# anitasyang/Laplace-GNN

Measured on AMD Instinct MI355X. Metric: la.fit() samples/sec (GCN, KFAC), higher is better.
Workload: dtype f32; 1 GPU; arxiv-shaped 2-layer GCN, hessian_structure=kron (BASELINE configs[2]); num_nodes=169343, nnz=2501719, features=128, hidden=256, classes=40, n_train=90941, batch_size=10000, batches=10, parallelism=dp1 ((batch, class) units, contiguous balanced runs)

## Files before the change

laplace-gnn_amd/csrc/batchcache.hip:

```cpp
#include "lgnn_internal.h"

#include <algorithm>
#include <cstdlib>

namespace lgnn {

namespace {

constexpr size_t kSeenMax = 256;

void free_entry_memory(BatchEntry* e) {
  const uint64_t tag = e->tag;
  const int64_t M = e->M;
  *e = BatchEntry{};
  e->tag = tag;
  e->M = M;
}

void remove_entry(lgnn_ctx* h, BatchEntry* e) {
  BatchCache& c = h->bcache;
  c.bytes -= e->bytes;
  c.entries.erase(std::find(c.entries.begin(), c.entries.end(), e));
  delete e;
}

bool make_room(lgnn_ctx* h, BatchEntry* e, size_t add, size_t budget) {
  BatchCache& c = h->bcache;
  if (e->bytes + add > budget) return false;
  while (c.bytes + add > budget) {
    BatchEntry* lru = nullptr;
    for (BatchEntry* o : c.entries)
      if (o != e && o->bytes > 0 && (!lru || o->last_use < lru->last_use)) lru = o;
    if (!lru) return false;
    remove_entry(h, lru);
  }
  return true;
}

template <class T>
int alloc_copy(DevArray<T>& dst, const void* src, size_t count, hipStream_t s) {
  dst = {};
  const size_t bytes = std::max<size_t>(count, 1) * sizeof(T);
  if (hipMalloc(&dst.buf.p, bytes) != hipSuccess) {
    (void)hipGetLastError();
    dst.buf.p = nullptr;
    return 1;
  }
  dst.buf.bytes = bytes;
  if (count > 0) LGNN_HIP_CHECK(hipMemcpyAsync(dst.buf.p, src, count * sizeof(T), hipMemcpyDeviceToDevice, s));
  return 0;
}

void refuse(lgnn_ctx* h, BatchEntry* e) {
  h->bcache.bytes -= e->bytes;
  free_entry_memory(e);
  e->refused = true;
}

}

size_t batch_cache_budget() {
  const char* e = getenv("LGNN_BATCH_CACHE_MB");
  const long long mb = e ? atoll(e) : 2048;
  return mb <= 0 ? 0 : size_t(mb) << 20;
}

void batch_cache_clear(lgnn_ctx* h) {
  BatchCache& c = h->bcache;
  for (BatchEntry* e : c.entries) delete e;
  c.entries.clear();
  c.seen.clear();
  c.bytes = 0;
}

void batch_cache_drop_tag(lgnn_ctx* h, uint64_t tag) {
  BatchCache& c = h->bcache;
  for (BatchEntry* e : c.entries)
    if (e->tag == tag) { remove_entry(h, e); break; }
  c.seen.erase(std::remove(c.seen.begin(), c.seen.end(), tag), c.seen.end());
}

int batch_cache_lookup(lgnn_ctx* h, uint64_t tag, const int64_t* idx, int64_t M, BatchEntry** out, hipStream_t s) {
  *out = nullptr;
  BatchCache& c = h->bcache;
  if (tag == 0) return 0;
  const size_t budget = batch_cache_budget();
  if (budget == 0) {
    if (!c.entries.empty() || !c.seen.empty()) batch_cache_clear(h);
    return 0;
  }
  while (c.bytes > budget) {
    BatchEntry* lru = nullptr;
    for (BatchEntry* o : c.entries)
      if (o->bytes > 0 && (!lru || o->last_use < lru->last_use)) lru = o;
    if (!lru) break;
    remove_entry(h, lru);
  }
  for (BatchEntry* e : c.entries)
    if (e->tag == tag) {
      if (e->M != M) { remove_entry(h, e); break; }
      if (e->refused) return 0;
      e->last_use = ++c.clock;
      *out = e;
      return 0;
    }
  auto it = std::find(c.seen.begin(), c.seen.end(), tag);
  if (it == c.seen.end()) {
    if (c.seen.size() >= kSeenMax) c.seen.erase(c.seen.begin());
    c.seen.push_back(tag);
    return 0;
  }
  c.seen.erase(it);
  BatchEntry* e = new (std::nothrow) BatchEntry();
  if (!e) return 0;
  e->tag = tag;
  e->M = M;
  e->last_use = ++c.clock;
  c.entries.push_back(e);
  const size_t add = size_t(M) * 8;
  if (!make_room(h, e, add, budget) || alloc_copy(e->ids, idx, size_t(M), s) != 0) { refuse(h, e); return 0; }
  e->bytes += add;
  c.bytes += add;
  *out = e;
  return 0;
}

int batch_cache_store_active(lgnn_ctx* h, BatchEntry* e, hipStream_t s) {
  if (e->has_act || e->refused) return 0;
  const int64_t N = h->N;
  int32_t n = 0;
  LGNN_HIP_CHECK(hipMemcpyAsync(&n, h->ws.act_count.p, 4, hipMemcpyDeviceToHost, s));
  LGNN_HIP_CHECK(hipStreamSynchronize(s));
  LGNN_REQUIRE(n >= 0 && n <= N, "internal: active-row count out of range");
  const size_t add = size_t(N) + size_t(std::max(n, 1)) * 4 + 4;
  if (!make_room(h, e, add, batch_cache_budget()) || alloc_copy(e->active, h->ws.active.p, size_t(N), s) != 0 ||
      alloc_copy(e->act_list, h->ws.act_list.p, size_t(n), s) != 0 ||
      alloc_copy(e->act_count, h->ws.act_count.p, 1, s) != 0) {
    refuse(h, e);
    return 0;
  }
  e->bytes += add;
  h->bcache.bytes += add;
  e->has_act = true;
  return 0;
}

int batch_cache_store_paths(lgnn_ctx* h, BatchEntry* e, int64_t cap, bool have_nodes, hipStream_t s) {
  if (e->has_paths || e->refused) return 0;
  const int64_t N = h->N;
  Workspace& ws = h->ws;
  int32_t cnt[3] = {0, 0, 0};
  LGNN_HIP_CHECK(hipMemcpyAsync(&cnt[0], ws.path_pptr.as<int32_t>() + N, 4, hipMemcpyDeviceToHost, s));
  LGNN_HIP_CHECK(hipMemcpyAsync(&cnt[1], ws.path_rptr.as<int32_t>() + N, 4, hipMemcpyDeviceToHost, s));
  if (have_nodes) LGNN_HIP_CHECK(hipMemcpyAsync(&cnt[2], ws.path_nnodes.p, 4, hipMemcpyDeviceToHost, s));
  LGNN_HIP_CHECK(hipStreamSynchronize(s));
  const size_t np = (cnt[0] >= 0 && int64_t(cnt[0]) <= cap) ? size_t(cnt[0]) : 0;
  LGNN_REQUIRE(cnt[1] >= 0 && int64_t(cnt[1]) <= std::max<int64_t>(h->nnz, 1) && cnt[2] >= 0 && cnt[2] <= N,
               "internal: path structure counts out of range");
  const size_t nr = size_t(cnt[1]), nn = size_t(cnt[2]);
  size_t add = size_t(N + 1) * 4 + std::max<size_t>(np, 1) * 12;
  add += size_t(N + 1) * 4 + std::max<size_t>(nr, 1) * 8;
  if (have_nodes) add += std::max<size_t>(nn, 1) * 4 + 4;
  bool ok = make_room(h, e, add, batch_cache_budget());
  ok = ok && alloc_copy(e->pptr, ws.path_pptr.p, size_t(N + 1), s) == 0 && alloc_copy(e->pm, ws.path_pm.p, np, s) == 0 &&
       alloc_copy(e->pv, ws.path_pv.p, np, s) == 0 && alloc_copy(e->pw, ws.path_pw.p, np, s) == 0;
  if (ok)
    ok = alloc_copy(e->rptr, ws.path_rptr.p, size_t(N + 1), s) == 0 && alloc_copy(e->r_m, ws.path_rm.p, nr, s) == 0 &&
         alloc_copy(e->r_w, ws.path_rw.p, nr, s) == 0;
  if (ok && have_nodes)
    ok = alloc_copy(e->nodes, ws.path_nodes.p, nn, s) == 0 && alloc_copy(e->nnodes, ws.path_nnodes.p, 1, s) == 0;
  if (!ok) { refuse(h, e); return 0; }
  e->bytes += add;
  h->bcache.bytes += add;
  e->path_bytes = add;
  e->cap = cap;
  e->has_nodes = have_nodes;
  e->has_paths = true;
  return 0;
}

int batch_cache_store_pairs(lgnn_ctx* h, BatchEntry* e, hipStream_t s) {
  if (e->has_pairs || e->pairs_refused || e->refused || !e->has_paths) return 0;
  const int64_t N = h->N;
  Workspace& ws = h->ws;
  int32_t np = 0;
  LGNN_HIP_CHECK(hipMemcpyAsync(&np, ws.pair_ptr.as<int32_t>() + N, 4, hipMemcpyDeviceToHost, s));
  LGNN_HIP_CHECK(hipStreamSynchronize(s));
  LGNN_REQUIRE(np >= 0 && size_t(np) * 4 <= ws.pair_m.bytes, "internal: pair count out of range");
  const size_t M = size_t(e->M), add = M * 4 + std::max<size_t>(size_t(np), 1) * 12 + 4;
  const bool ok = make_room(h, e, add, batch_cache_budget()) && alloc_copy(e->pair_s, ws.pair_s.p, M, s) == 0 &&
                  alloc_copy(e->pair_m, ws.pair_m.p, size_t(np), s) == 0 && alloc_copy(e->pair_m2, ws.pair_m2.p, size_t(np), s) == 0 &&
                  alloc_copy(e->pair_w, ws.pair_w.p, size_t(np), s) == 0 &&
                  alloc_copy(e->pair_n, ws.pair_ptr.as<int32_t>() + N, 1, s) == 0;
  if (!ok) {
    e->pair_s = {}; e->pair_m = {}; e->pair_m2 = {}; e->pair_w = {}; e->pair_n = {};
    e->pairs_refused = true;
    return 0;
  }
  e->bytes += add;
  h->bcache.bytes += add;
  e->path_bytes += add;
  e->has_pairs = true;
  return 0;
}

void batch_cache_drop_paths(lgnn_ctx* h, BatchEntry* e) {
  if (!e->has_paths) return;
  e->pair_s = {}; e->pair_m = {}; e->pair_m2 = {}; e->pair_w = {}; e->pair_n = {};
  e->has_pairs = e->pairs_refused = false;
  e->pptr = {}; e->pm = {}; e->pv = {}; e->pw = {}; e->nodes = {}; e->nnodes = {}; e->rptr = {}; e->r_m = {}; e->r_w = {};
  e->has_paths = e->has_nodes = false;
  h->bcache.bytes -= e->path_bytes;
  e->bytes -= e->path_bytes;
  e->path_bytes = 0;
}

}

using namespace lgnn;

extern "C" int lgnn_kfac_batch_tag(lgnn_ctx* h, uint64_t tag) {
  if (!h) { set_error("null context"); return 2; }
  h->bcache.pending_tag = tag;
  return 0;
}

extern "C" int lgnn_batch_cache_drop(lgnn_ctx* h, uint64_t tag) {
  if (!h) { set_error("null context"); return 2; }
  if (tag == 0) batch_cache_clear(h);
  else batch_cache_drop_tag(h, tag);
  return 0;
}

extern "C" int lgnn_batch_cache_stats(const lgnn_ctx* h, int64_t* out) {
  if (!h || !out) { set_error("null argument"); return 2; }
  const BatchCache& c = h->bcache;
  int64_t n = 0;
  for (const BatchEntry* e : c.entries) n += e->bytes > 0 ? 1 : 0;
  out[0] = n; out[1] = int64_t(c.bytes); out[2] = c.hits; out[3] = c.misses; out[4] = c.builds;
  return 0;
}
```

laplace-gnn_amd/csrc/lgnn_internal.h:

```cpp
#pragma once
#include <atomic>
#include <cstring>
#include <hip/hip_runtime.h>
#include <stdint.h>
#include <string>
#include <type_traits>
#include <vector>

#include "../../include/laplace_gnn_hip.h"

namespace lgnn {

void set_error(const std::string& msg);

#define LGNN_HIP_CHECK(expr)                                                              \
  do {                                                                                    \
    hipError_t _e = (expr);                                                               \
    if (_e != hipSuccess) {                                                               \
      lgnn::set_error(std::string(#expr) + ": " + hipGetErrorString(_e));                 \
      return 1;                                                                           \
    }                                                                                     \
  } while (0)

#define LGNN_REQUIRE(cond, msg)                                                           \
  do {                                                                                    \
    if (!(cond)) {                                                                        \
      lgnn::set_error(std::string(msg) + " (" #cond ")");                                 \
      return 2;                                                                           \
    }                                                                                     \
  } while (0)

#define LGNN_CALL(expr)                                                                   \
  do {                                                                                    \
    int _rc = (expr);                                                                     \
    if (_rc != 0) return _rc;                                                             \
  } while (0)

inline int64_t cdiv(int64_t a, int64_t b) { return (a + b - 1) / b; }

template <auto Kernel>
int lds_opt_in(int bytes) {
  static std::atomic<uint64_t> done{0};
  int dev = 0;
  LGNN_HIP_CHECK(hipGetDevice(&dev));
  const uint64_t bit = dev < 64 ? uint64_t(1) << dev : 0;
  if (done.load(std::memory_order_acquire) & bit) return 0;
  LGNN_HIP_CHECK(hipFuncSetAttribute(reinterpret_cast<const void*>(Kernel), hipFuncAttributeMaxDynamicSharedMemorySize, bytes));
  done.fetch_or(bit, std::memory_order_release);
  return 0;
}

struct DevBuf {
  void* p = nullptr;
  size_t bytes = 0;
  bool host = false;
  DevBuf() = default;
  ~DevBuf();
  DevBuf(const DevBuf&) = delete;
  DevBuf& operator=(const DevBuf&) = delete;
  DevBuf(DevBuf&& o) noexcept;
  DevBuf& operator=(DevBuf&& o) noexcept;
  int reserve(size_t want);
  int reserve_host(size_t want);
  void release();
  template <class T> T* as() const { return reinterpret_cast<T*>(p); }
};
static_assert(!std::is_copy_constructible_v<DevBuf>);

struct Csr {
  int32_t* rowptr = nullptr;
  int32_t* col = nullptr;
  float* val = nullptr;
};

constexpr int kMaxLayers = 8;

struct ForwardCache {
  bool valid = false;
  bool aux_valid = false;
  bool wt_valid = false;
  bool x_valid = false;
  bool px_valid = false;
  DevBuf Xpad;
  int64_t prop_ld[kMaxLayers] = {};
  bool gram_valid[kMaxLayers] = {};
  DevBuf lin_in[kMaxLayers];
  DevBuf act_out[kMaxLayers];
  const float* lin_in_p[kMaxLayers] = {};
  int64_t lin_in_ld[kMaxLayers] = {};
  const float* hact_p[kMaxLayers] = {};
  int64_t hact_ld[kMaxLayers] = {};
  DevBuf out;
  DevBuf tmp;
  DevBuf gram_raw[kMaxLayers];
  DevBuf prop_in[kMaxLayers];
  DevBuf rowsum;
  DevBuf dact0;
  DevBuf mask_bits[kMaxLayers];
  DevBuf xhat[kMaxLayers];
  DevBuf rstd[kMaxLayers];
  DevBuf res_out;
  DevBuf pre_norm;
  template <class F> void each_buf(F&& f) const {
    for (int l = 0; l < kMaxLayers; ++l) {
      f(lin_in[l]); f(act_out[l]); f(gram_raw[l]); f(prop_in[l]); f(mask_bits[l]); f(xhat[l]); f(rstd[l]);
    }
    f(Xpad); f(out); f(tmp); f(rowsum); f(dact0); f(res_out); f(pre_norm);
  }
};

struct Workspace {
  DevBuf pos;
  DevBuf seeds;
  DevBuf probs;
  DevBuf mult;
  DevBuf planes_a;
  const void* planes_a_zero_ptr = nullptr;
  size_t planes_a_zero_bytes = 0;
  DevBuf planes_b;
  DevBuf gram_scratch[kMaxLayers];
  DevBuf misc;
  DevBuf jac;
  DevBuf top;
  DevBuf active;
  DevBuf val_act;
  DevBuf act_list;
  DevBuf act_count;
  DevBuf select_tmp;
  DevBuf flags;
  DevBuf out_flags, out_list, out_count;
  DevBuf val_act2;
  DevBuf path_coef, path_up, path_bg, path_cnt, path_rptr, path_rm, path_rw, path_zeros;
  DevBuf path_alpha;
  DevBuf path_pcnt, path_pptr, path_pm, path_pv, path_pw;
  DevBuf path_flags, path_nodes, path_nnodes;
  DevBuf pair_s, pair_cnt, pair_ptr, pair_m, pair_m2, pair_w;
  DevBuf pair_part;
  bool path_zeros_set = false;
  DevBuf gram_scratch_res[kMaxLayers];
  DevBuf planes_c;
  DevBuf adj_z0;
  DevBuf adj_dir;
  DevBuf lora_rows, lora_cols, lora_state, lora_count, lora_part;
  DevBuf dense_stored;
  DevBuf dense_rows;
  DevBuf subnet_keys, subnet_ord, subnet_iota, subnet_tmp, subnet_plan, subnet_x;
  DevBuf gp_tab_a, gp_tab_b, gp_phi_a, gp_phi_b, gp_g, gp_kt, gp_s, gp_wpair, gp_part, gp_jac_a, gp_jac_b;
  DevBuf cov_phit_a, cov_phit_b, cov_phis, cov_t2, cov_va, cov_vb, cov_add, cov_small, cov_scr;
  DevBuf ggn_jac, ggn_u, ggn_wt, ggn_tmp;
  DevBuf ggn_q, ggn_qbar, ggn_part;
  DevBuf cand_rows, cand_ord, cand_iota, cand_tmp, cand_ptr;
  template <class F> void each_buf(F&& f) const {
    for (int l = 0; l < kMaxLayers; ++l) { f(gram_scratch[l]); f(gram_scratch_res[l]); }
    f(pos); f(seeds); f(probs); f(mult); f(planes_a); f(planes_b); f(misc); f(jac); f(top); f(active); f(val_act);
    f(act_list); f(act_count); f(select_tmp); f(flags); f(out_flags); f(out_list); f(out_count); f(val_act2);
    f(path_coef); f(path_up); f(path_bg); f(path_cnt); f(path_rptr); f(path_rm); f(path_rw); f(path_zeros); f(path_alpha);
    f(path_pcnt); f(path_pptr); f(path_pm); f(path_pv); f(path_pw); f(path_flags); f(path_nodes); f(path_nnodes);
    f(pair_s); f(pair_cnt); f(pair_ptr); f(pair_m); f(pair_m2); f(pair_w); f(pair_part);
    f(planes_c); f(adj_z0); f(adj_dir); f(lora_rows); f(lora_cols); f(lora_state); f(lora_count); f(lora_part);
    f(dense_stored); f(dense_rows);
    f(subnet_keys); f(subnet_ord); f(subnet_iota); f(subnet_tmp); f(subnet_plan); f(subnet_x);
    f(gp_tab_a); f(gp_tab_b); f(gp_phi_a); f(gp_phi_b); f(gp_g); f(gp_kt); f(gp_s); f(gp_wpair); f(gp_part); f(gp_jac_a);
    f(gp_jac_b); f(cov_phit_a); f(cov_phit_b); f(cov_phis); f(cov_t2); f(cov_va); f(cov_vb); f(cov_add); f(cov_small);
    f(cov_scr); f(ggn_jac); f(ggn_u); f(ggn_wt); f(ggn_tmp); f(ggn_q); f(ggn_qbar); f(ggn_part);
    f(cand_rows); f(cand_ord); f(cand_iota); f(cand_tmp); f(cand_ptr);
  }
};

template <class T>
struct DevArray {
  DevBuf buf;
  operator T*() const { return buf.as<T>(); }
};
struct BatchEntry {
  uint64_t tag = 0;
  int64_t M = 0;
  uint64_t last_use = 0;
  size_t bytes = 0, path_bytes = 0;
  bool refused = false;
  DevArray<int64_t> ids;
  bool has_act = false;
  DevArray<uint8_t> active;
  DevArray<int32_t> act_list;
  DevArray<int32_t> act_count;
  bool has_paths = false;
  int64_t cap = 0;
  DevArray<int32_t> pptr;
  DevArray<int32_t> pm;
  DevArray<int32_t> pv;
  DevArray<float> pw;
  bool has_nodes = false;
  DevArray<int32_t> nodes;
  DevArray<int32_t> nnodes;
  DevArray<int32_t> rptr;
  DevArray<int32_t> r_m;
  DevArray<float> r_w;
  bool has_pairs = false;
  bool pairs_refused = false;
  DevArray<float> pair_s;
  DevArray<int32_t> pair_m;
  DevArray<int32_t> pair_m2;
  DevArray<float> pair_w;
  DevArray<int32_t> pair_n;
};
struct BatchCache {
  std::vector<BatchEntry*> entries;
  std::vector<uint64_t> seen;
  uint64_t pending_tag = 0;
  uint64_t clock = 0;
  size_t bytes = 0;
  int64_t hits = 0, misses = 0, builds = 0;
};

struct TrainState {
  bool tape_valid = false;
  bool input_valid = false;
  int64_t M = 0;
  float scale = 1.f;
  const uint8_t* masks[kMaxLayers] = {};
  DevBuf in[kMaxLayers];
  DevBuf xhat[kMaxLayers];
  DevBuf rstd[kMaxLayers];
  DevBuf out;
  DevBuf z, res;
  DevBuf ga, gb;
  DevBuf keys, keys_sorted, ord, ord_sorted, sort_tmp;
  DevBuf part;
  DevBuf wstack;
  DevBuf norm_part;
  template <class F> void each_buf(F&& f) const {
    for (int l = 0; l < kMaxLayers; ++l) { f(in[l]); f(xhat[l]); f(rstd[l]); }
    f(out); f(z); f(res); f(ga); f(gb); f(keys); f(keys_sorted); f(ord); f(ord_sorted); f(sort_tmp);
    f(part); f(wstack); f(norm_part);
  }
};

struct SampledState {
  bool in_valid = false;
  int64_t ldk = 0;
  DevBuf in0;
  DevBuf need;
  DevBuf rows;
  DevBuf count;
  DevBuf rpos;
  DevBuf z;
  DevBuf select_tmp;
  template <class F> void each_buf(F&& f) const {
    f(in0); f(need); f(rows); f(count); f(rpos); f(z); f(select_tmp);
  }
};

}

struct lgnn_ctx {
  int64_t N = 0;
  int64_t nnz = 0;
  int kind = 0;
  bool sym = false;
  bool self_loops = false;
  lgnn::Csr A, AT;
  lgnn::DevBuf A_rowptr, A_col, AT_rowptr, AT_col, val_fwd, val_bwd, deg_scale;
  lgnn::Csr P, PT;
  int L = 0;
  int64_t dims[lgnn::kMaxLayers + 1] = {};
  int64_t in_dim[lgnn::kMaxLayers] = {};
  const float* W[lgnn::kMaxLayers] = {};
  const float* b[lgnn::kMaxLayers] = {};
  const float* X = nullptr;
  int act = 0, lik = 0;
  int64_t n_params = 0;
  lgnn::DevBuf Wt[lgnn::kMaxLayers];
  bool has_res = false;
  int norm = 0;
  float norm_eps = 1e-5f;
  const float* Wr[lgnn::kMaxLayers] = {};
  const float* br[lgnn::kMaxLayers] = {};
  const float* norm_w[lgnn::kMaxLayers] = {};
  const float* norm_b[lgnn::kMaxLayers] = {};
  const float* norm_mean[lgnn::kMaxLayers] = {};
  const float* norm_var[lgnn::kMaxLayers] = {};
  lgnn::DevBuf Wrt[lgnn::kMaxLayers];
  lgnn::DevBuf Wcomb[lgnn::kMaxLayers], bcomb[lgnn::kMaxLayers];
  bool extras() const { return has_res || norm != 0; }
  int n_blocks() const { return has_res ? 2 * L - 1 : L; }
  const float* Wback(int l) const {
    return (has_res && kind == LGNN_KIND_SAGE && l < L - 1) ? Wcomb[l].as<float>() : W[l];
  }
  lgnn::ForwardCache fc;
  lgnn::Workspace ws;
  int64_t ws_limit = int64_t(32) << 30;
  int64_t cov_chunk_pairs = 0;
  bool last_route_paths = false;
  int last_top_kernel = 0;
  double two_hop_max = -1.0;
  double pair_hop_max = -1.0;
  double two_hop = -1.0;
  int64_t n_long = -1;
  int64_t n_long_tasks = 0;
  lgnn::DevBuf long_rows, long_slot, long_tasks, hub;
  lgnn::DevBuf top_multi, top_tasks, top_task_count, top_cnt, top_offs, top_hub_tiles;
  int64_t n_top_multi = 0, n_top_slices = 0;
  int64_t n_long_fwd = -1;
  lgnn::DevBuf long_rows_fwd;
  bool timing = false;
  std::vector<hipEvent_t> ev;
  size_t ev_used = 0;
  int64_t ev_planes = 0;
  lgnn::BatchCache bcache;
  lgnn::TrainState tr;
  lgnn::SampledState sf;
  template <class F> void each_buf(F&& f) const {
    for (int l = 0; l < lgnn::kMaxLayers; ++l) { f(Wt[l]); f(Wrt[l]); f(Wcomb[l]); f(bcomb[l]); }
    f(A_rowptr); f(A_col); f(AT_rowptr); f(AT_col); f(val_fwd); f(val_bwd); f(deg_scale);
    f(long_rows); f(long_slot); f(long_tasks); f(hub); f(long_rows_fwd);
    f(top_multi); f(top_tasks); f(top_task_count); f(top_cnt); f(top_offs); f(top_hub_tiles);
    fc.each_buf(f); ws.each_buf(f); tr.each_buf(f); sf.each_buf(f);
  }
  ~lgnn_ctx();
};

namespace lgnn {

struct SpmmArgs {
  const int32_t* rowptr;
  const int32_t* col;
  const float* val;
  int64_t nrows;
  const float* in;
  int64_t in_ld;
  int64_t in_plane_stride;
  float* out;
  int64_t out_ld;
  int64_t out_plane_stride;
  int64_t width;
  const float* self;
  int64_t self_ld;
  int64_t self_plane_stride;
  const float* hact;
  int64_t hact_ld;
  int act;
  int out_act;
  const int32_t* long_rows; int64_t n_long;
  bool skip_zero;
};

struct FusedArgs {
  const int32_t* rowptr; const int32_t* col; const float* val;
  int64_t nrows;
  int64_t nplanes;
  const float* in; int64_t in_ld; int64_t in_plane_stride;
  float* store; int64_t store_ld; int64_t store_plane_stride;
  const float* self; int64_t self_ld; int64_t self_plane_stride;
  const float* hact; int64_t hact_ld; int act;
  const uint8_t* self_rows; const uint32_t* mask_bits; int mask_words;
  int64_t width;
  float* scratch;
  int unused_;
  const int32_t* long_slot; const float* hub; int64_t hub_plane_stride; int64_t n_long;
  const int32_t* row_list; const int32_t* row_count;
};

struct BackGemmArgs {
  const float* G;
  const float* W;
  int64_t ldw;
  float* U;
  int64_t u_plane_stride;
  int64_t N, K, Nout;
  int64_t planes;
  const int32_t* rows;
  const int32_t* na_dev;
  const uint32_t* mask_bits; int64_t mask_words;
  const float* hact; int64_t hact_ld; int act;
};
bool backgemm_supported(int64_t K, int64_t Nout, bool with_mask);
int launch_backgemm(const BackGemmArgs& g, hipStream_t s);
int launch_relu_mask_bits(const float* h, int64_t ld, int64_t N, int64_t H, uint32_t* bits, hipStream_t s);
int compact_flags(const uint8_t* flags, int64_t n, int32_t* out, int32_t* count_dev, DevBuf& tmp, hipStream_t s);
int compact_rows(lgnn_ctx* h, const uint8_t* flags, DevBuf& list, DevBuf& count, hipStream_t s);
int compact_active_rows(lgnn_ctx* h, hipStream_t s);
int kfac_top_planes(lgnn_ctx* h, const int64_t* idx, int64_t M, bool fork_exact, float* g, hipStream_t s);
int exclusive_scan_i32(int32_t* in, int32_t* out, int64_t n, DevBuf& tmp, hipStream_t s);

int graph_build(lgnn_ctx* h, const int64_t* edge_index, int64_t E, hipStream_t s);
int graph_values(lgnn_ctx* h, bool same, hipStream_t s);
int graph_update(lgnn_ctx* h, const int64_t* fi, const int64_t* fj, const uint8_t* st, int64_t K, hipStream_t s);

struct DenseNtArgs {
  float* out = nullptr;
  int64_t ldo = 0, ncols = 0, nrows = 0;
  const int32_t* nrows_dev = nullptr;
  const int32_t* orows = nullptr;
  const int32_t* lrows = nullptr;
  const float* L = nullptr;
  int64_t l_ld = 0, l_stride = 0;
  const float* R = nullptr;
  int64_t r_ld = 0, r_stride = 0;
  int64_t width = 0, nplanes = 1;
  const float* rowc = nullptr;
  int64_t rowc_ld = 0;
};
int launch_dense_nt(const DenseNtArgs& g, hipStream_t s);
int launch_dense_diag_pair(const int64_t* idx, int64_t m0, int64_t mc, int64_t N, const int32_t* pos, const int32_t* mult,
                           const float* mask, int64_t H, const float* PX, int64_t ldx, const float* rowsum, int64_t F,
                           const float* H1p, int64_t ldh, const float* T, const float* phibar, float* out, hipStream_t s);
int launch_gp_rowcol(lgnn_ctx* h, const float* gP, float* rs, float* cs, hipStream_t s);
int dense_adj_finish(lgnn_ctx* h, float* G, hipStream_t s);

int launch_spmm(const Csr& m, int64_t nrows, const float* in, int64_t in_ld, float* out, int64_t out_ld,
                int64_t width, int epilogue, hipStream_t s, const int32_t* long_rows = nullptr, int64_t n_long = 0);
int launch_csr_rowsum(const Csr& m, int64_t nrows, float* out, hipStream_t s);

struct GemmEpilogue {
  const float* bias = nullptr;
  const float* hact = nullptr;
  int64_t hact_ld = 0;
  int act = 0;
  int64_t hact_row_mod = 0;
  int out_act = -1;
  const uint8_t* row_active = nullptr;
  bool no_atomics = false;
};
int launch_gemm(const float* A, int64_t lda, const float* B, int64_t ldb, float* C, int64_t ldc, int64_t R,
                int64_t K, int64_t Nout, const GemmEpilogue& ep, hipStream_t s);
int launch_gemm_devrows(const float* A, int64_t lda, const float* B, int64_t ldb, float* C, int64_t ldc, int64_t rows_bound,
                        const int32_t* r_dev, int64_t r_mul, int64_t K, int64_t Nout, float alpha, hipStream_t s);
int launch_gemm_listed(const float* A, int64_t lda, const float* B, int64_t ldb, float* C, int64_t ldc, int64_t planes,
                       int64_t plane_rows, const int32_t* list, const int32_t* na_dev, int64_t K, int64_t Nout,
                       const GemmEpilogue& ep, hipStream_t s);

int launch_gram(const float* X, int64_t ld, int64_t R, int64_t D, float* scratch, hipStream_t s);
int launch_gram_scaled(const float* X, int64_t ld, int64_t R, int64_t D, float* out, float scale, hipStream_t s);
int launch_gram_batched(const float* X, int64_t ld, int64_t R, int64_t D, float* out, int64_t out_zstride, int64_t nz,
                        const float* row_scale, const float* zscale, float scale, hipStream_t s);
int launch_symmetrize_upper(float* H, int64_t D, hipStream_t s);
int launch_sym_accumulate(const float* scratch, int64_t D, float scale, float* out, hipStream_t s, int64_t scratch_ld = 0);
int launch_spmm_ex(const SpmmArgs& a, int64_t nplanes, hipStream_t s);
int launch_spmm_gram_ex(const FusedArgs& a, hipStream_t s);
int launch_spmm_gram256(const FusedArgs& a, hipStream_t s);
bool fused_supported(int64_t width, int64_t in_ld, int64_t in_plane_stride, const void* in, int64_t rows);
int launch_spmm_gram(const Csr& m, int64_t nrows, int64_t nplanes, const float* in, float* store_or_null,
                     int64_t width, float* scratch, hipStream_t s);

int launch_transpose(const float* in, int64_t rows, int64_t cols, float* out, hipStream_t s);
int launch_act_deriv(const float* h, int64_t ld, int64_t N, int64_t H, int act, float* out, hipStream_t s);
int launch_fill_i32(int32_t* p, int64_t n, int32_t v, hipStream_t s);
int launch_gather_rows(const float* in, int64_t ld, int64_t nrows_in, const int64_t* idx, int64_t M, int64_t width,
                       float* out, int* bad_flag, hipStream_t s);

int launch_norm_forward(lgnn_ctx* h, int layer, const float* spre, int64_t s_ld, float* out, int64_t out_ld, hipStream_t s);
int launch_resnorm_backward(lgnn_ctx* h, int layer, float* U, int64_t ld, int64_t rows, const float* add, bool mask,
                            hipStream_t s);
int build_sage_res_weights(lgnn_ctx* h, int layer, hipStream_t s);
constexpr int kLongRow = 64;
constexpr int kTopSlice = 128;
int long_rows_ensure(lgnn_ctx* h, hipStream_t s);
int long_rows_fwd_ensure(lgnn_ctx* h, hipStream_t s);
int launch_long_rows_spmm(lgnn_ctx* h, const float* val, const float* in, int64_t in_ld, int64_t in_plane_stride,
                          int64_t nplanes, int64_t width, hipStream_t s);
struct KfacPlan {
  bool seeds_on_the_fly;
  bool sage_compact;
  bool need_pong;
  bool paths;
  bool fuse[kMaxLayers];
  bool backgemm[kMaxLayers];
  int64_t maxw, cc_max;
};
KfacPlan plan_kfac(int kind, int L, int64_t N, int64_t nnz, const int64_t* dims, int act, bool no_fuse, int64_t ws_limit,
                   bool no_paths = false);
struct KfacFisherOpts {
  const void* y_seed;
  float resid_scale;
  float b_scale;
  bool add_loss_and_A;
};
struct KfacShare { int64_t begin, end, count; };
int kfac_accumulate(lgnn_ctx* h, const int64_t* idx, const void* y, int64_t M, int64_t n_train, uint32_t flags,
                    int64_t class_begin, int64_t class_end, float* const* A_out, float* const* B_out, float* loss_out,
                    hipStream_t s, const KfacFisherOpts* fisher = nullptr, const KfacShare* share = nullptr);
int batch_prologue(lgnn_ctx* h, const int64_t* idx, const void* y, int64_t M, bool want_seeds, bool fork_exact,
                   float* loss_out, hipStream_t s, const void* y_seed = nullptr, float resid_scale = 1.0f,
                   const int64_t* guard_ids = nullptr);
int batch_epilogue(lgnn_ctx* h, const int64_t* idx, int64_t M, hipStream_t s);
int record_event(lgnn_ctx* h, hipStream_t s);
size_t batch_cache_budget();
void batch_cache_clear(lgnn_ctx* h);
int batch_cache_lookup(lgnn_ctx* h, uint64_t tag, const int64_t* idx, int64_t M, BatchEntry** out, hipStream_t s);
int batch_cache_store_active(lgnn_ctx* h, BatchEntry* e, hipStream_t s);
int batch_cache_store_paths(lgnn_ctx* h, BatchEntry* e, int64_t cap, bool have_nodes, hipStream_t s);
int batch_cache_store_pairs(lgnn_ctx* h, BatchEntry* e, hipStream_t s);
void batch_cache_drop_paths(lgnn_ctx* h, BatchEntry* e);
int launch_gram256_stream(const float* Y, int64_t ld, int64_t rows, int64_t width, float* scratch, hipStream_t s,
                          const int32_t* gate = nullptr, int64_t gate_cap = 0);
bool paths_supported(int kind, int L, const int64_t* dims, int act, int64_t nnz);
int two_hop_ensure(lgnn_ctx* h, hipStream_t s);
bool paths_pay(const lgnn_ctx* h, int64_t M);
constexpr int kCoefStride = 64;
constexpr int kCoefRow = 256;
struct PathR { const int32_t* rptr; const int32_t* r_m; const float* r_w; };
int launch_top_tiles(lgnn_ctx* h, const PathR& r, int64_t M, int64_t cb, int64_t ce, const int32_t* act_list,
                     const int32_t* act_count, float* scratch, hipStream_t s);
struct TopPairs { const float* sq; const int32_t* pm; const int32_t* pm2; const float* pw; const int32_t* npairs; };
int64_t top_pairs_bound(const lgnn_ctx* h, int64_t M);
bool top_pairs_fit(const lgnn_ctx* h, int64_t M);
int build_top_pairs(lgnn_ctx* h, const int64_t* idx, int64_t M, const PathR& r, TopPairs& out, hipStream_t s);
int launch_top_pairs(lgnn_ctx* h, const TopPairs& p, int64_t M, int64_t cb, int64_t ce, float* scratch, hipStream_t s);
struct TopTilesReq { const int32_t* act_list; const int32_t* act_count; float* scratch; bool pairs; };
int kfac_paths_first_layer(lgnn_ctx* h, const int64_t* idx, int64_t M, int seed_mode, int64_t cb, int64_t ce, float* scratch,
                           hipStream_t s, int64_t nb = 0, int64_t ne = -1, BatchEntry* entry = nullptr, bool* built = nullptr,
                           const TopTilesReq* top = nullptr);
int kfac_paths_first_layer_sage(lgnn_ctx* h, const int64_t* idx, int64_t M, int seed_mode, int64_t cb, int64_t ce,
                                float* scratch, hipStream_t s, int64_t nb = 0, int64_t ne = -1);
int forward_ensure(lgnn_ctx* h, hipStream_t s);
int forward_ensure_grams(lgnn_ctx* h, hipStream_t s);
int forward_ensure_aux(lgnn_ctx* h, hipStream_t s);
int forward_input_view(lgnn_ctx* h, hipStream_t s);
int build_px(lgnn_ctx* h, hipStream_t s);
int ensure_wt(lgnn_ctx* h, hipStream_t s);
bool gcn2_small_forward_supported(const lgnn_ctx* h);
int gcn2_forward_through_px(lgnn_ctx* h, hipStream_t s);
int diag_accumulate(lgnn_ctx* h, const int64_t* idx, const void* y, int64_t M, uint32_t flags, float* diag_out,
                    float* loss_out, hipStream_t s);
int lastlayer_full_accumulate(lgnn_ctx* h, const int64_t* idx, const void* y, int64_t M, float* H_out,
                              float* loss_out, hipStream_t s);
int lastlayer_pairs_accumulate(lgnn_ctx* h, const int64_t* idx, const void* y, int64_t M, float* S, float* Sb,
                               float* loss_out, hipStream_t s);
int lastlayer_features(lgnn_ctx* h, const int64_t* idx, int64_t M, float* out, float* f_out, hipStream_t s);
int lastlayer_pairs_place(lgnn_ctx* h, const float* S, const float* Sb, float* H_out, hipStream_t s);
int ef_accumulate(lgnn_ctx* h, const int64_t* idx, const void* y_seed, const void* y_loss, int64_t M, float resid_scale,
                  float scale, float* diag_out, float* full_out, float* grads_out, float* loss_out, hipStream_t s);
int lastlayer_kron_accumulate(lgnn_ctx* h, const int64_t* idx, const void* y, int64_t M, int64_t n_train, uint32_t flags,
                              float* A_out, float* B_out, float* Bb_out, float* loss_out, hipStream_t s);
int lastlayer_diag_accumulate(lgnn_ctx* h, const int64_t* idx, const void* y, int64_t M, float* diag_out, float* loss_out,
                              hipStream_t s);
int jacobians(lgnn_ctx* h, const int64_t* idx, int64_t M, float* J, float* f_out, hipStream_t s);
int full_accumulate(lgnn_ctx* h, const int64_t* idx, const void* y, int64_t M, float* H_out, float* loss_out, hipStream_t s);
int jacobians_subset(lgnn_ctx* h, const int64_t* idx, int64_t M, const int64_t* subnet, int64_t S, float* J, float* f_out,
                     hipStream_t s);
int subnet_full_accumulate(lgnn_ctx* h, const int64_t* idx, const void* y, int64_t M, const int64_t* subnet, int64_t S,
                           float* H_out, float* loss_out, hipStream_t s);
int gp_kernel(lgnn_ctx* h, const int64_t* idx_a, int64_t Ma, const int64_t* idx_b, int64_t Mb, int flags, float* K, int64_t ldk,
              hipStream_t s);
int gp_jvp(lgnn_ctx* h, const int64_t* idx, int64_t M, const float* v, float* out, hipStream_t s);
int glm_covariance(lgnn_ctx* h, const int64_t* idx_a, int64_t Ma, const int64_t* idx_b, int64_t Mb, int n_blocks,
                   const float* const* QA, const float* const* QB, const float* const* S, int flags, float* K, int64_t ldk,
                   hipStream_t s);
struct NtProblem {
  const float* A; int64_t lda, a_bs;
  const float* B; int64_t ldb, b_bs;
  float* Out; int64_t ldo, o_es, o_bs;
  int64_t Ra, Rb, K, batch;
  int upper_only = 0;
};
int launch_nt_gemm(lgnn_ctx* h, const NtProblem& p, hipStream_t s);
int jvp_block(lgnn_ctx* h, const int64_t* idx, int64_t M, const float* V, int64_t k, float* out, hipStream_t s);
int ggn_matmat(lgnn_ctx* h, const int64_t* idx, const void* y, int64_t M, const float* V, int64_t k, int flags, float* G,
               float* loss_out, hipStream_t s);
int sampled_forward(lgnn_ctx* h, const int64_t* idx, int64_t M, const float* theta, int64_t S, uint32_t flags, float* out,
                    hipStream_t s);
int sampled_ensure_input(lgnn_ctx* h, hipStream_t s);
int sampled_needed_rows(lgnn_ctx* h, const int64_t* idx, int64_t M, hipStream_t s);
struct GatherArgs {
  const int64_t* idx; int64_t M, N;
  const int32_t* rowptr; const int32_t* col; const float* val;
  const int32_t* rpos;
  const float* z; int64_t rcap, Cz, C;
  int sage, cw;
  const float* theta; int64_t P, offb;
  int64_t ns;
  float* out;
};
int launch_sampled_gather(const GatherArgs& g, hipStream_t s);
constexpr int SBM = 64, SBH = 64, SBK = 64, SLDT = SBK + 1, SLDH = SBH + 1, SZW = 128;
struct FwdArgs {
  static constexpr bool linearised = true;
  const float* in0; int64_t ldk;
  const int32_t* rows; const int32_t* count;
  const float* theta; int64_t P;
  int64_t Fp, H;
  const float* dact; const float* h1; int64_t h1_ld;
  const float* W1; int64_t ld1, off1, C, Cz;
  float* z; int64_t rcap;
};
int launch_first_layer(const FwdArgs& a, bool two, int64_t ndir, hipStream_t s);
int launch_full_directions(const float* J, const float* Gamma, const int64_t* idx, const float* logits, int64_t N,
                           int64_t mc, int64_t C, int64_t P, float* R, float* Kn, hipStream_t s);
void* blas_handle(hipStream_t s);
int sgemm_rm(hipStream_t s, int64_t R, int64_t Nout, int64_t K, float alpha, const float* A, int64_t lda, const float* B,
             int64_t ldb, float beta, float* Cm, int64_t ldc);

}
```

laplace-gnn_amd/csrc/paths.h:

```cpp
#pragma once
#include "lgnn_internal.h"

namespace lgnn {

constexpr int kYRows = 48;
__device__ __forceinline__ int coef_slot(int rel) { return ((rel & 15) << 2) | (rel >> 4); }
__device__ __forceinline__ int slot_class(int slot) { return ((slot & 3) << 4) | (slot >> 2); }
using f32x4 = __attribute__((ext_vector_type(4))) float;

struct YArgs {
  const int32_t* rowptr; const int32_t* col; const float* val;
  const int32_t* rptr; const int32_t* r_m; const float* r_w;
  const int32_t* pptr; const int32_t* pm; const int32_t* pv; const float* pw;
  int64_t cap;
  const float* coef;
  const float* zeros;
  const float* bg;
  const uint32_t* mask;
  int mask_words;
  const float* W1;
  int w1_ld;
  float* Y;
  int64_t N, M;
  int64_t n0, n1;
  const int32_t* list;
  const int32_t* n_list;
  int H, c0, R;
  int cb;
  int64_t n_coef;
  int unused_;
  int no_bg;
  int gram_f32;
};
static_assert(sizeof(YArgs) == 240 && __builtin_offsetof(YArgs, no_bg) == 228, "YArgs: paths_fused_kernel's argument offsets");

struct PathLists {
  const int32_t* rptr; const int32_t* r_m; const float* r_w;
  const int32_t* pptr; const int32_t* pm; const int32_t* pv; const float* pw;
  const int32_t* nodes; const int32_t* nnodes;
};

int launch_paths_fused(lgnn_ctx* h, YArgs y, int64_t cb, int64_t ce, float* scratch, hipStream_t s);
int launch_paths_overflow(lgnn_ctx* h, YArgs y, int64_t cb, int64_t ce, float* scratch, hipStream_t s);

}
```

laplace-gnn_amd/csrc/paths.hip:

```cpp
#include "device_utils.h"
#include "paths.h"

namespace lgnn {

namespace {

__global__ __launch_bounds__(256) void path_tables_kernel(const float* __restrict__ probs, const float* __restrict__ logits,
                                                          const int64_t* __restrict__ idx, const int32_t* __restrict__ pos,
                                                          int64_t M, int64_t N, int C, int cb, int ce, int mode,
                                                          float* __restrict__ coef, float* __restrict__ up,
                                                          const float* __restrict__ W1, int H, float* __restrict__ bg) {
  const int lane = threadIdx.x & 63;
  const int64_t m = int64_t(blockIdx.x) * 4 + (threadIdx.x >> 6);
  if (m >= M) return;
  const int64_t n = idx[m];
  float* __restrict__ cm = coef + m * kCoefRow;
  float* __restrict__ um = up + m * C;
  float* __restrict__ pm = up + (M + m) * C;
  const bool own = n >= 0 && n < N && pos[n] == int32_t(m);
  float pk = 0.f, fk = 0.f;
  if (own && lane < C && mode != 2) { pk = probs[m * C + lane]; fk = logits[n * C + lane]; }
  const float mb = wave_sum(pk * fk);
  const float sp = sqrtf(pk), t = fk - mb;
  float al = 0.f, be = 0.f, ga = 0.f, u = 0.f;
  if (own && lane < C) {
    if (mode == 2) al = 1.41421356237309515f;
    else if (mode == 1) { al = sp * (1.f + 0.5f * t); be = sp; ga = 0.5f * sp * t; u = pk * (1.f + t); }
    else { al = sp; be = sp; u = pk; }
  }
  const int c = cb + slot_class(lane);
  const bool have = c < ce;
  const int src = have ? c : 0;
  const float sal = __shfl(al, src), sbe = __shfl(be, src), sga = __shfl(ga, src);
  cm[lane] = have ? sal : 0.f;
  cm[kCoefStride + lane] = have ? -sbe : 0.f;
  cm[2 * kCoefStride + lane] = have ? -sga : 0.f;
  cm[3 * kCoefStride + lane] = 0.f;
  if (lane < C) { um[lane] = u; pm[lane] = own ? pk : 0.f; }
  if (bg == nullptr) return;
  const bool colv = 4 * lane < H;
  f32x4 b4 = {0.f, 0.f, 0.f, 0.f}, g4 = {0.f, 0.f, 0.f, 0.f};
  if (own) {
    const float* __restrict__ w = W1 + (colv ? 4 * lane : 0);
    for (int c = 0; c < C; ++c) {
      const float uc = __int_as_float(__builtin_amdgcn_readlane(__float_as_int(u), c));
      const float pc = __int_as_float(__builtin_amdgcn_readlane(__float_as_int(pk), c));
      const f32x4 wc = *reinterpret_cast<const f32x4*>(w + int64_t(c) * H);
      b4 += uc * wc;
      g4 += pc * wc;
    }
  }
  if (colv) {
    *reinterpret_cast<f32x4*>(bg + m * H + 4 * lane) = b4;
    *reinterpret_cast<f32x4*>(bg + (M + m) * H + 4 * lane) = g4;
  }
}

template <bool FILL>
__global__ __launch_bounds__(256) void path_r_kernel(const int64_t* __restrict__ idx, int64_t M, int64_t N,
                                                     const int32_t* __restrict__ pos, const int32_t* __restrict__ mult,
                                                     const int32_t* __restrict__ rowptr, const int32_t* __restrict__ col,
                                                     const float* __restrict__ val, int32_t* __restrict__ cnt,
                                                     const int32_t* __restrict__ rptr, int32_t* __restrict__ r_m,
                                                     float* __restrict__ r_w) {
  const int lane = threadIdx.x & 63;
  const int64_t m = int64_t(blockIdx.x) * 4 + (threadIdx.x >> 6);
  if (m >= M) return;
  const int64_t u = idx[m];
  if (u < 0 || u >= N || pos[u] != int32_t(m)) return;
  const float tm = FILL ? float(mult[m]) : 0.f;
  const int32_t e = rowptr[u + 1];
  for (int32_t p = rowptr[u] + lane; p < e; p += 64) {
    const int32_t v = col[p];
    const int32_t k = atomicAdd(&cnt[v], 1);
    if constexpr (FILL) {
      const int32_t slot = rptr[v] + k;
      r_m[slot] = int32_t(m);
      r_w[slot] = val[p] * tm;
    }
  }
}

template <bool FILL>
__global__ __launch_bounds__(256) void path_list_kernel(const int32_t* __restrict__ rowptr, const int32_t* __restrict__ col,
                                                        const float* __restrict__ val, int64_t N,
                                                        const int32_t* __restrict__ rptr, const int32_t* __restrict__ r_m,
                                                        const float* __restrict__ r_w, int32_t* __restrict__ pcnt,
                                                        const int32_t* __restrict__ pptr, int64_t cap,
                                                        int32_t* __restrict__ pm, int32_t* __restrict__ pv,
                                                        float* __restrict__ pw) {
  const int lane = threadIdx.x & 63;
  const int64_t n = int64_t(blockIdx.x) * 4 + (threadIdx.x >> 6);
  if (n >= N) return;
  if constexpr (FILL) {
    if (int64_t(pptr[N]) > cap) return;
  }
  const int32_t s = rowptr[n], e = rowptr[n + 1];
  int32_t run = FILL ? pptr[n] : 0;
  for (int32_t base = s; base < e; base += 64) {
    int32_t v = 0, r0 = 0, cnt = 0;
    float pval = 0.f;
    if (base + lane < e) {
      v = col[base + lane];
      pval = val[base + lane];
      r0 = rptr[v];
      cnt = rptr[v + 1] - r0;
    }
    int incl = cnt;
#pragma unroll
    for (int o = 1; o < 64; o <<= 1) {
      const int t = __shfl_up(incl, o);
      if (lane >= o) incl += t;
    }
    if constexpr (FILL) {
      const int32_t off = run + incl - cnt;
      for (int k = 0; k < cnt; ++k) {
        pm[off + k] = r_m[r0 + k];
        pv[off + k] = v;
        pw[off + k] = pval * r_w[r0 + k];
      }
    }
    run += __shfl(incl, 63);
  }
  if (!FILL && lane == 0) pcnt[n] = run;
}

__global__ __launch_bounds__(256) void sage_path_tables_kernel(const float* __restrict__ probs, const float* __restrict__ logits,
                                                               const int64_t* __restrict__ idx, const int32_t* __restrict__ pos,
                                                               int64_t M, int64_t N, int C, int cb, int ce, int mode,
                                                               float* __restrict__ coef, float* __restrict__ up,
                                                               float* __restrict__ alpha) {
  const int lane = threadIdx.x & 63;
  const int64_t m = int64_t(blockIdx.x) * 4 + (threadIdx.x >> 6);
  if (m >= M + C) return;
  const int c = cb + slot_class(lane);
  const bool have = c < ce;
  if (m >= M) {
    float* __restrict__ cm = coef + (2 * M + (m - M)) * kCoefRow;
    cm[lane] = 0.f; cm[kCoefStride + lane] = (have && c == int(m - M)) ? 1.f : 0.f; cm[2 * kCoefStride + lane] = 0.f; cm[3 * kCoefStride + lane] = 0.f;
    return;
  }
  const int64_t n = idx[m];
  const bool own = n >= 0 && n < N && pos[n] == int32_t(m);
  float pk = 0.f, fk = 0.f;
  if (own && lane < C && mode != 2) { pk = probs[m * C + lane]; fk = logits[n * C + lane]; }
  const float mb = wave_sum(pk * fk);
  const float sp = sqrtf(pk), t = fk - mb;
  float al = 0.f, be = 0.f, ga = 0.f, u = 0.f;
  if (own && lane < C) {
    if (mode == 2) al = 1.41421356237309515f;
    else if (mode == 1) { al = sp * (1.f + 0.5f * t); be = sp; ga = 0.5f * sp * t; u = pk * (1.f + t); }
    else { al = sp; be = sp; u = pk; }
  }
  const int src = have ? c : 0;
  float sal = __shfl(al, src), sbe = __shfl(be, src), sga = __shfl(ga, src);
  if (!have) { sal = 0.f; sbe = 0.f; sga = 0.f; }
  float* __restrict__ cs = coef + (2 * m) * kCoefRow;
  float* __restrict__ cn = coef + (2 * m + 1) * kCoefRow;
  cs[lane] = 0.f; cs[kCoefStride + lane] = -sbe; cs[2 * kCoefStride + lane] = -sga; cs[3 * kCoefStride + lane] = 0.f;
  cn[lane] = sal; cn[kCoefStride + lane] = -sbe; cn[2 * kCoefStride + lane] = -sga; cn[3 * kCoefStride + lane] = 0.f;
  alpha[m * kCoefStride + lane] = al;
  if (lane < C) { up[m * C + lane] = u; up[(M + m) * C + lane] = own ? pk : 0.f; }
}

template <bool FILL>
__global__ __launch_bounds__(256) void sage_path_list_kernel(const int32_t* __restrict__ rowptr, const int32_t* __restrict__ col,
                                                             const float* __restrict__ val, int64_t N, int64_t M, int C,
                                                             const int32_t* __restrict__ pos, const int32_t* __restrict__ mult,
                                                             const float* __restrict__ alpha, int32_t* __restrict__ pcnt,
                                                             const int32_t* __restrict__ pptr, int32_t* __restrict__ pm,
                                                             int32_t* __restrict__ pv, float* __restrict__ pw) {
  const int lane = threadIdx.x & 63;
  const int64_t n = int64_t(blockIdx.x) * 4 + (threadIdx.x >> 6);
  if (n >= N) return;
  const int32_t s = rowptr[n], e = rowptr[n + 1];
  int32_t run = FILL ? pptr[n] : 0;
  for (int32_t base = s; base < e; base += 64) {
    int32_t mv = INT32_MAX;
    float w = 0.f;
    if (base + lane < e) { mv = pos[col[base + lane]]; w = val[base + lane]; }
    const bool in = mv != INT32_MAX;
    const uint64_t bal = __ballot(in);
    if constexpr (FILL) {
      if (in) {
        const int32_t o = run + __popcll(bal & ((uint64_t(1) << lane) - 1));
        pm[o] = 2 * mv + 1; pv[o] = int32_t(n); pw[o] = w * float(mult[mv]);
      }
    }
    run += __popcll(bal);
  }
  const int32_t ms = pos[n];
  if (ms != INT32_MAX) {
    if constexpr (FILL) {
      const float tm = float(mult[ms]);
      if (lane == 0) { pm[run] = 2 * ms; pv[run] = int32_t(n); pw[run] = tm; }
      if (lane < C) {
        pm[run + 1 + lane] = int32_t(2 * M) + lane; pv[run + 1 + lane] = int32_t(n);
        pw[run + 1 + lane] = tm * alpha[int64_t(ms) * kCoefStride + lane];
      }
    }
    run += 1 + C;
  }
  if (!FILL && lane == 0) pcnt[n] = run;
}

__global__ void path_flag_kernel(const int32_t* __restrict__ pptr, int64_t n0, int64_t n, uint8_t* __restrict__ flags) {
  const int64_t k = int64_t(blockIdx.x) * blockDim.x + threadIdx.x;
  if (k < n) flags[k] = pptr[n0 + k + 1] > pptr[n0 + k] ? 1 : 0;
}

__global__ void two_hop_count_kernel(const int32_t* __restrict__ rp, const int32_t* __restrict__ rpt, int64_t N,
                                     unsigned long long* __restrict__ out) {
  unsigned long long acc = 0;
  const int64_t stride = int64_t(gridDim.x) * blockDim.x;
  for (int64_t v = int64_t(blockIdx.x) * blockDim.x + threadIdx.x; v < N; v += stride)
    acc += (unsigned long long)(rp[v + 1] - rp[v]) * (unsigned long long)(rpt[v + 1] - rpt[v]);
  for (int o = 32; o > 0; o >>= 1) acc += __shfl_xor(acc, o);
  if ((threadIdx.x & 63) == 0 && acc) atomicAdd(out, acc);
}

__global__ void two_hop_max_kernel(const int32_t* __restrict__ rp, const int32_t* __restrict__ col,
                                   const int32_t* __restrict__ rp2, int64_t N, unsigned long long* __restrict__ out) {
  unsigned long long best = 0;
  const int64_t stride = int64_t(gridDim.x) * blockDim.x;
  for (int64_t m = int64_t(blockIdx.x) * blockDim.x + threadIdx.x; m < N; m += stride) {
    unsigned long long acc = 0;
    for (int32_t p = rp[m]; p < rp[m + 1]; ++p) { const int32_t k = col[p]; acc += (unsigned long long)(rp2[k + 1] - rp2[k]); }
    best = acc > best ? acc : best;
  }
  for (int o = 32; o > 0; o >>= 1) { const unsigned long long t = __shfl_xor(best, o); best = t > best ? t : best; }
  if ((threadIdx.x & 63) == 0 && best) atomicMax(out, best);
}
}

int two_hop_ensure(lgnn_ctx* h, hipStream_t s) {
  if (h->two_hop >= 0) return 0;
  h->two_hop = 0;
  if (h->nnz <= 0) return 0;
  DevBuf acc;
  LGNN_CALL(acc.reserve(64));
  unsigned long long host[3] = {0, 0, 0};
  LGNN_HIP_CHECK(hipMemsetAsync(acc.p, 0, 24, s));
  const dim3 grid{unsigned(std::min<int64_t>(cdiv(h->N, 256), 1024))};
  hipLaunchKernelGGL(two_hop_count_kernel, grid, dim3(256), 0, s, h->P.rowptr, h->PT.rowptr, h->N, acc.as<unsigned long long>());
  LGNN_HIP_CHECK(hipGetLastError());
  hipLaunchKernelGGL(two_hop_max_kernel, grid, dim3(256), 0, s, h->P.rowptr, h->P.col, h->P.rowptr, h->N,
                     acc.as<unsigned long long>() + 1);
  LGNN_HIP_CHECK(hipGetLastError());
  hipLaunchKernelGGL(two_hop_max_kernel, grid, dim3(256), 0, s, h->P.rowptr, h->P.col, h->PT.rowptr, h->N,
                     acc.as<unsigned long long>() + 2);
  LGNN_HIP_CHECK(hipGetLastError());
  LGNN_HIP_CHECK(hipMemcpyAsync(host, acc.p, 24, hipMemcpyDeviceToHost, s));
  LGNN_HIP_CHECK(hipStreamSynchronize(s));
  h->two_hop = double(host[0]);
  h->two_hop_max = double(host[1]);
  h->pair_hop_max = double(host[2]);
  return 0;
}
constexpr double kPathsPerNodeLimit = 24.0;
bool paths_pay(const lgnn_ctx* h, int64_t M) {
  const double N = double(h->N);
  return h->two_hop >= 0 && h->two_hop / N * double(M) / N <= kPathsPerNodeLimit;
}

bool paths_supported(int kind, int L, const int64_t* dims, int act, int64_t nnz) {
  const int64_t C = dims[L], H = L >= 2 ? dims[L - 1] : 0;
  return (kind == LGNN_KIND_GCN || kind == LGNN_KIND_SAGE) && L == 2 && act == LGNN_ACT_RELU && nnz > 0 && C <= kCoefStride &&
         H > 128 && H <= 256 && H % 4 == 0;
}

static int64_t path_list_cap(const lgnn_ctx* h) {
  int64_t cap = std::max<int64_t>(4 * h->nnz, int64_t(1) << 22);
  if (const char* e = getenv("LGNN_PATH_LIST_CAP")) cap = std::max<int64_t>(1, std::min<int64_t>(cap, atoll(e)));
  return cap;
}
bool top_pairs_fit(const lgnn_ctx* h, int64_t M) {
  int64_t cap = path_list_cap(h);
  if (const char* e = getenv("LGNN_PAIR_LIST_CAP")) cap = std::max<int64_t>(1, std::min<int64_t>(cap, atoll(e)));
  const int64_t bound = top_pairs_bound(h, M);
  return bound > 0 && bound <= cap;
}

static int path_node_list(lgnn_ctx* h, PathLists& pl, int64_t nb, int64_t ne, hipStream_t s) {
  Workspace& ws = h->ws;
  const int64_t n = ne - nb;
  LGNN_CALL(ws.path_flags.reserve(size_t(h->N)));
  LGNN_CALL(ws.path_nodes.reserve(size_t(h->N) * 4));
  LGNN_CALL(ws.path_nnodes.reserve(64));
  hipLaunchKernelGGL(path_flag_kernel, dim3(unsigned(cdiv(n, 256))), dim3(256), 0, s, pl.pptr, nb, n, ws.path_flags.as<uint8_t>());
  LGNN_HIP_CHECK(hipGetLastError());
  pl.nodes = ws.path_nodes.as<int32_t>(); pl.nnodes = ws.path_nnodes.as<int32_t>();
  return compact_flags(ws.path_flags.as<uint8_t>(), n, ws.path_nodes.as<int32_t>(), ws.path_nnodes.as<int32_t>(), ws.select_tmp, s);
}
static int path_list_reserve(lgnn_ctx* h, int64_t cap, PathLists& pl, hipStream_t s) {
  Workspace& ws = h->ws;
  LGNN_CALL(ws.path_pcnt.reserve(size_t(h->N + 1) * 4));
  LGNN_CALL(ws.path_pptr.reserve(size_t(h->N + 1) * 4));
  LGNN_CALL(ws.path_pm.reserve(size_t(cap) * 4));
  LGNN_CALL(ws.path_pv.reserve(size_t(cap) * 4));
  LGNN_CALL(ws.path_pw.reserve(size_t(cap) * 4));
  LGNN_HIP_CHECK(hipMemsetAsync(ws.path_pcnt.as<int32_t>() + h->N, 0, 4, s));
  pl.pptr = ws.path_pptr.as<int32_t>(); pl.pm = ws.path_pm.as<int32_t>(); pl.pv = ws.path_pv.as<int32_t>();
  pl.pw = ws.path_pw.as<float>();
  return 0;
}
static int path_zeros_ensure(Workspace& ws, hipStream_t s) {
  LGNN_CALL(ws.path_zeros.reserve(1024));
  if (!ws.path_zeros_set) LGNN_HIP_CHECK(hipMemsetAsync(ws.path_zeros.p, 0, 1024, s));
  ws.path_zeros_set = true;
  return 0;
}

static YArgs path_args(lgnn_ctx* h, const PathLists& pl, int64_t cb, int64_t cap, int64_t nb, int64_t ne) {
  YArgs y{};
  y.rowptr = h->PT.rowptr; y.col = h->PT.col; y.val = h->PT.val;
  y.rptr = pl.rptr; y.r_m = pl.r_m; y.r_w = pl.r_w;
  y.pptr = pl.pptr; y.pm = pl.pm; y.pv = pl.pv; y.pw = pl.pw; y.cap = cap;
  y.list = pl.nodes; y.n_list = pl.nnodes;
  y.coef = h->ws.path_coef.as<float>(); y.bg = h->ws.path_bg.as<float>(); y.zeros = h->ws.path_zeros.as<float>();
  y.mask = h->fc.mask_bits[0].as<uint32_t>(); y.mask_words = int(cdiv(h->dims[1], 32));
  y.N = h->N; y.n0 = nb; y.n1 = ne; y.H = int(h->dims[1]); y.cb = int(cb);
  return y;
}

int kfac_paths_first_layer(lgnn_ctx* h, const int64_t* idx, int64_t M, int seed_mode, int64_t cb, int64_t ce, float* scratch,
                           hipStream_t s, int64_t nb, int64_t ne, BatchEntry* entry, bool* built, const TopTilesReq* top) {
  const int64_t N = h->N, C = h->dims[2], H = h->dims[1];
  if (ne < 0) ne = N;
  LGNN_REQUIRE(nb >= 0 && nb <= ne && ne <= N, "internal: node range");
  if (nb == ne) return 0;
  Workspace& ws = h->ws;
  LGNN_REQUIRE(paths_supported(h->kind, h->L, h->dims, h->act, h->nnz), "internal: path route on an unsupported model");
  LGNN_CALL(ws.path_coef.reserve(size_t(M) * kCoefRow * 4));
  LGNN_CALL(ws.path_up.reserve(size_t(2 * M) * C * 4));
  LGNN_CALL(ws.path_bg.reserve(size_t(2 * M) * H * 4));
  const bool no_bg = seed_mode == 2;
  const bool bg_in_tables = !no_bg && (reinterpret_cast<uintptr_t>(h->W[1]) & 15) == 0;
  hipLaunchKernelGGL(path_tables_kernel, dim3(unsigned(cdiv(M, 4))), dim3(256), 0, s, ws.probs.as<float>(),
                     h->fc.out.as<float>(), idx, ws.pos.as<int32_t>(), M, N, int(C), int(cb), int(ce), seed_mode,
                     ws.path_coef.as<float>(), ws.path_up.as<float>(), h->W[1], int(H),
                     bg_in_tables ? ws.path_bg.as<float>() : static_cast<float*>(nullptr));
  LGNN_HIP_CHECK(hipGetLastError());
  if (!no_bg && !bg_in_tables) {
    GemmEpilogue none;
    LGNN_CALL(launch_gemm(ws.path_up.as<float>(), C, h->W[1], H, ws.path_bg.as<float>(), H, 2 * M, C, H, none, s));
  }
  const int64_t cap = path_list_cap(h);
  const bool can_overflow = !(h->two_hop_max >= 0 && double(M) * h->two_hop_max <= double(cap));
  const double ppn = h->two_hop >= 0 ? h->two_hop / double(N) * double(M) / double(N) : 1e9;
  const bool use_list = ppn < 2.5;
  const bool whole = nb == 0 && ne == N;
  LGNN_CALL(path_zeros_ensure(ws, s));
  if (entry && entry->refused) entry = nullptr;
  if (entry && entry->has_paths && entry->cap != cap) batch_cache_drop_paths(h, entry);
  const bool cached = entry && entry->has_paths;
  PathLists pl{};
  if (cached) {
    pl = {entry->rptr, entry->r_m, entry->r_w, entry->pptr, entry->pm, entry->pv, entry->pw, nullptr, nullptr};
  } else {
    LGNN_CALL(ws.path_cnt.reserve(size_t(N + 1) * 4));
    LGNN_CALL(ws.path_rptr.reserve(size_t(N + 1) * 4));
    LGNN_CALL(ws.path_rm.reserve(size_t(std::max<int64_t>(h->nnz, 1)) * 4));
    LGNN_CALL(ws.path_rw.reserve(size_t(std::max<int64_t>(h->nnz, 1)) * 4));
    LGNN_HIP_CHECK(hipMemsetAsync(ws.path_cnt.p, 0, size_t(N + 1) * 4, s));
    hipLaunchKernelGGL(path_r_kernel<false>, dim3(unsigned(cdiv(M, 4))), dim3(256), 0, s, idx, M, N, ws.pos.as<int32_t>(),
                       ws.mult.as<int32_t>(), h->P.rowptr, h->P.col, h->P.val, ws.path_cnt.as<int32_t>(),
                       static_cast<const int32_t*>(nullptr), static_cast<int32_t*>(nullptr), static_cast<float*>(nullptr));
    LGNN_HIP_CHECK(hipGetLastError());
    LGNN_CALL(exclusive_scan_i32(ws.path_cnt.as<int32_t>(), ws.path_rptr.as<int32_t>(), N + 1, ws.select_tmp, s));
    LGNN_HIP_CHECK(hipMemsetAsync(ws.path_cnt.p, 0, size_t(N + 1) * 4, s));
    hipLaunchKernelGGL(path_r_kernel<true>, dim3(unsigned(cdiv(M, 4))), dim3(256), 0, s, idx, M, N, ws.pos.as<int32_t>(),
                       ws.mult.as<int32_t>(), h->P.rowptr, h->P.col, h->P.val, ws.path_cnt.as<int32_t>(),
                       ws.path_rptr.as<int32_t>(), ws.path_rm.as<int32_t>(), ws.path_rw.as<float>());
    LGNN_HIP_CHECK(hipGetLastError());
    LGNN_CALL(path_list_reserve(h, cap, pl, s));
    const dim3 pgrid{unsigned(cdiv(N, 4))};
    hipLaunchKernelGGL(path_list_kernel<false>, pgrid, dim3(256), 0, s, h->PT.rowptr, h->PT.col, h->PT.val, N,
                       ws.path_rptr.as<int32_t>(), ws.path_rm.as<int32_t>(), ws.path_rw.as<float>(), ws.path_pcnt.as<int32_t>(),
                       static_cast<const int32_t*>(nullptr), cap, static_cast<int32_t*>(nullptr), static_cast<int32_t*>(nullptr),
                       static_cast<float*>(nullptr));
    LGNN_HIP_CHECK(hipGetLastError());
    LGNN_CALL(exclusive_scan_i32(ws.path_pcnt.as<int32_t>(), ws.path_pptr.as<int32_t>(), N + 1, ws.select_tmp, s));
    hipLaunchKernelGGL(path_list_kernel<true>, pgrid, dim3(256), 0, s, h->PT.rowptr, h->PT.col, h->PT.val, N,
                       ws.path_rptr.as<int32_t>(), ws.path_rm.as<int32_t>(), ws.path_rw.as<float>(), ws.path_pcnt.as<int32_t>(),
                       ws.path_pptr.as<int32_t>(), cap, ws.path_pm.as<int32_t>(), ws.path_pv.as<int32_t>(), ws.path_pw.as<float>());
    LGNN_HIP_CHECK(hipGetLastError());
    pl.rptr = ws.path_rptr.as<int32_t>(); pl.r_m = ws.path_rm.as<int32_t>(); pl.r_w = ws.path_rw.as<float>();
  }
  if (use_list) {
    if (cached && whole && entry->has_nodes) {
      pl.nodes = entry->nodes; pl.nnodes = entry->nnodes;
    } else {
      LGNN_CALL(path_node_list(h, pl, nb, ne, s));
    }
  }
  if (entry && !cached) {
    LGNN_CALL(batch_cache_store_paths(h, entry, cap, use_list && whole, s));
    if (built) *built = true;
  }
  if (top && top->pairs) {
    TopPairs tp{};
    if (entry && entry->has_pairs) {
      tp = {entry->pair_s, entry->pair_m, entry->pair_m2, entry->pair_w, entry->pair_n};
    } else {
      LGNN_CALL(build_top_pairs(h, idx, M, PathR{pl.rptr, pl.r_m, pl.r_w}, tp, s));
      if (entry && entry->has_paths) LGNN_CALL(batch_cache_store_pairs(h, entry, s));
    }
    LGNN_CALL(launch_top_pairs(h, tp, M, cb, ce, top->scratch, s));
  } else if (top) {
    LGNN_CALL(launch_top_tiles(h, PathR{pl.rptr, pl.r_m, pl.r_w}, M, cb, ce, top->act_list, top->act_count, top->scratch, s));
  }
  YArgs y = path_args(h, pl, cb, cap, nb, ne);
  y.W1 = h->W[1]; y.w1_ld = int(H); y.M = M; y.n_coef = M; y.no_bg = no_bg ? 1 : 0;
  LGNN_CALL(launch_paths_fused(h, y, cb, ce, scratch, s));
  return can_overflow ? launch_paths_overflow(h, y, cb, ce, scratch, s) : 0;
}

int kfac_paths_first_layer_sage(lgnn_ctx* h, const int64_t* idx, int64_t M, int seed_mode, int64_t cb, int64_t ce, float* scratch,
                                hipStream_t s, int64_t nb, int64_t ne) {
  const int64_t N = h->N, C = h->dims[2], H = h->dims[1];
  if (ne < 0) ne = N;
  LGNN_REQUIRE(nb >= 0 && nb <= ne && ne <= N, "internal: node range");
  if (nb == ne) return 0;
  Workspace& ws = h->ws;
  LGNN_REQUIRE(h->kind == LGNN_KIND_SAGE && paths_supported(h->kind, h->L, h->dims, h->act, h->nnz),
               "internal: path route on an unsupported model");
  const int64_t T = 2 * M + C;
  LGNN_CALL(ws.path_coef.reserve(size_t(T) * kCoefRow * 4));
  LGNN_CALL(ws.path_up.reserve(size_t(2 * M) * C * 4));
  LGNN_CALL(ws.path_bg.reserve(size_t(2 * T) * H * 4));
  LGNN_CALL(ws.path_alpha.reserve(size_t(M) * kCoefStride * 4));
  hipLaunchKernelGGL(sage_path_tables_kernel, dim3(unsigned(cdiv(M + C, 4))), dim3(256), 0, s, ws.probs.as<float>(),
                     h->fc.out.as<float>(), idx, ws.pos.as<int32_t>(), M, N, int(C), int(cb), int(ce), seed_mode,
                     ws.path_coef.as<float>(), ws.path_up.as<float>(), ws.path_alpha.as<float>());
  LGNN_HIP_CHECK(hipGetLastError());
  float* bg = ws.path_bg.as<float>();
  GemmEpilogue none;
  LGNN_CALL(launch_gemm(ws.path_up.as<float>(), C, h->W[1], 2 * H, bg, 2 * H, M, C, 2 * H, none, s));
  LGNN_CALL(launch_gemm(ws.path_up.as<float>() + M * C, C, h->W[1], 2 * H, bg + T * H, 2 * H, M, C, 2 * H, none, s));
  LGNN_HIP_CHECK(hipMemcpy2DAsync(bg + 2 * M * H, size_t(H) * 4, h->W[1], size_t(2 * H) * 4, size_t(H) * 4, size_t(C),
                                  hipMemcpyDeviceToDevice, s));
  LGNN_HIP_CHECK(hipMemsetAsync(bg + (T + 2 * M) * H, 0, size_t(C) * H * 4, s));
  LGNN_CALL(path_zeros_ensure(ws, s));
  const int64_t cap = std::max<int64_t>(h->nnz, 1) + (C + 1) * M + 64;
  LGNN_REQUIRE(cap < (int64_t(1) << 31), "too many paths for one launch");
  PathLists pl{};
  LGNN_CALL(path_list_reserve(h, cap, pl, s));
  const dim3 pgrid{unsigned(cdiv(N, 4))};
  hipLaunchKernelGGL(sage_path_list_kernel<false>, pgrid, dim3(256), 0, s, h->PT.rowptr, h->PT.col, h->PT.val, N, M, int(C),
                     ws.pos.as<int32_t>(), ws.mult.as<int32_t>(), ws.path_alpha.as<float>(), ws.path_pcnt.as<int32_t>(),
                     static_cast<const int32_t*>(nullptr), static_cast<int32_t*>(nullptr), static_cast<int32_t*>(nullptr),
                     static_cast<float*>(nullptr));
  LGNN_HIP_CHECK(hipGetLastError());
  LGNN_CALL(exclusive_scan_i32(ws.path_pcnt.as<int32_t>(), ws.path_pptr.as<int32_t>(), N + 1, ws.select_tmp, s));
  hipLaunchKernelGGL(sage_path_list_kernel<true>, pgrid, dim3(256), 0, s, h->PT.rowptr, h->PT.col, h->PT.val, N, M, int(C),
                     ws.pos.as<int32_t>(), ws.mult.as<int32_t>(), ws.path_alpha.as<float>(), ws.path_pcnt.as<int32_t>(),
                     ws.path_pptr.as<int32_t>(), ws.path_pm.as<int32_t>(), ws.path_pv.as<int32_t>(), ws.path_pw.as<float>());
  LGNN_HIP_CHECK(hipGetLastError());
  LGNN_CALL(path_node_list(h, pl, nb, ne, s));
  YArgs y = path_args(h, pl, cb, cap, nb, ne);
  y.W1 = h->W[1] + H; y.w1_ld = int(2 * H);
  y.M = T; y.n_coef = T; y.no_bg = 0;
  return launch_paths_fused(h, y, cb, ce, scratch, s);
}

}
```

laplace-gnn_amd/csrc/paths_fused.hip:

```cpp
#include "gram256.h"
#include "paths.h"

namespace lgnn {
namespace {

constexpr int kYStride = 272;
constexpr int kPlaneDwords = 512;
constexpr int kGroupDwords = 3 * kPlaneDwords;
constexpr int kYGroups = kYRows / 4;
__device__ __forceinline__ int piece_swap(int q) { return (q ^ (q >> 2)) & 1; }
__device__ __forceinline__ int piece_col(int c) { return 8 * (c >> 2) + 4 * (((c >> 1) & 1) ^ piece_swap(c >> 2)) + 2 * (c & 1); }

struct alignas(16) FusedShared {
  union {
    uint32_t pc[2][kYGroups][3][kPlaneDwords];
    float y[2][kYRows][kYStride];
  };
  int ready[4], done[4];
};
static_assert(sizeof(FusedShared) <= 160 * 1024, "the CU's LDS");

__device__ __forceinline__ int lds_min4(const int* c) {
  int4 v;
  asm volatile("ds_read_b128 %0, %1\n\ts_waitcnt lgkmcnt(0)" : "=v"(v) : "v"(uint32_t(reinterpret_cast<uintptr_t>(c))) : "memory");
  return __builtin_amdgcn_readfirstlane(min(min(v.x, v.y), min(v.z, v.w)));
}
__device__ __forceinline__ void lds_publish(int* c, int value, int lane) {
  if (lane == 0)
    asm volatile("ds_write_b32 %0, %1\n\ts_waitcnt lgkmcnt(0)" :: "v"(uint32_t(reinterpret_cast<uintptr_t>(c))), "v"(value) : "memory");
}

using i32x4 = int __attribute__((ext_vector_type(4)));
__device__ __forceinline__ i32x4 make_rsrc(const void* p, uint64_t bytes) {
  const uint64_t u = reinterpret_cast<uint64_t>(p);
  return i32x4{int(uint32_t(u)), int(uint32_t(u >> 32) & 0xffffu), int(uint32_t(bytes > 0xffffffffull ? 0xffffffffull : bytes)),
               0x00020000};
}
template <bool LIST>
struct NodeRanges {
  i32x4 prs, lrs;
  uint32_t r;
  int64_t base, cnt;
  uint32_t n0;
  __device__ __forceinline__ void init(const int32_t* __restrict__ pptr, const int32_t* __restrict__ list, int64_t n0_, int64_t N,
                                       int64_t nn, int64_t cnt_) {
    prs = make_rsrc(pptr, uint64_t(N + 1) * 4);
    lrs = make_rsrc(LIST ? list : pptr, uint64_t(LIST ? nn : 0) * 4);
    n0 = uint32_t(n0_); cnt = cnt_;
    fill(0);
  }
  __device__ __forceinline__ void fill(int64_t b) {
    base = b;
    const uint32_t ii = uint32_t(b) + (threadIdx.x & 31u);
    const bool in = int64_t(ii) < cnt;
    const uint32_t k = blockIdx.x + ii * gridDim.x;
    uint32_t node = k;
    if constexpr (LIST)
      asm volatile("buffer_load_dword %0, %1, %2, 0 offen\n\ts_waitcnt vmcnt(0)" : "=&v"(node) : "v"(in ? k * 4u : 0xfffffff0u), "s"(lrs) : "memory");
    const uint32_t off = in ? (n0 + node) * 4u + ((threadIdx.x >> 3) & 4u) : 0xfffffff0u;
    asm volatile("buffer_load_dword %0, %1, %2, 0 offen\n\ts_waitcnt vmcnt(0)" : "=&v"(r) : "v"(off), "s"(prs) : "memory");
  }
  __device__ __forceinline__ void get(int64_t i, int32_t& p0, int32_t& p1) {
    if (i - base >= 32) fill(i);
    const int l = int(i - base);
    p0 = __builtin_amdgcn_readlane(int(r), l); p1 = __builtin_amdgcn_readlane(int(r), l + 32);
  }
};

template <int OFF>
__device__ __forceinline__ void bload4(f32x4& d, uint32_t voff, const i32x4& rsrc) {
  asm volatile("buffer_load_dwordx4 %0, %1, %2, 0 offen offset:%3" : "=v"(d) : "v"(voff), "s"(rsrc), "n"(OFF) : "memory");
}
__device__ __forceinline__ void bload1(uint32_t& d, uint32_t voff, const i32x4& rsrc) {
  asm volatile("buffer_load_dword %0, %1, %2, 0 offen" : "=v"(d) : "v"(voff), "s"(rsrc) : "memory");
}
using bf16x8 = __attribute__((ext_vector_type(8))) __bf16;
using u32x4v = __attribute__((ext_vector_type(4))) uint32_t;
using u32x2v = __attribute__((ext_vector_type(2))) uint32_t;

__device__ __forceinline__ uint32_t pk_bf16(float lo, float hi) {
  using bf16x2 = __attribute__((ext_vector_type(2))) __bf16;
  const bf16x2 v = {static_cast<__bf16>(lo), static_cast<__bf16>(hi)};
  return __builtin_bit_cast(uint32_t, v);
}
__device__ __forceinline__ void split_pair(float ya, float yb, uint32_t& q0, uint32_t& q1, uint32_t& q2) {
  q0 = pk_bf16(ya, yb);
  asm("" : "+v"(q0));
  const float r1a = ya - __uint_as_float(q0 << 16), r1b = yb - __uint_as_float(q0 & 0xffff0000u);
  q1 = pk_bf16(r1a, r1b);
  asm("" : "+v"(q1));
  q2 = pk_bf16(r1a - __uint_as_float(q1 << 16), r1b - __uint_as_float(q1 & 0xffff0000u));
}

struct PTables {
  i32x4 coef, b, g, mask, pm, pv, pw;
};

struct PMeta { uint32_t oc, ob, om, w; };
__device__ __forceinline__ void meta_issue(const PTables& tb, int32_t p0, int32_t p1, int lane, PMeta& t) {
  const uint32_t q = uint32_t(max(min(p0 + lane, p1 - 1), 0)) * 4u;
  bload1(t.oc, q, tb.pm);
  bload1(t.om, q, tb.pv);
  bload1(t.w, q, tb.pw);
}
template <int YOUNGER>
__device__ __forceinline__ void meta_finish(int32_t p0, int32_t p1, int lane, uint32_t row_bytes, uint32_t mask_bytes, PMeta& t) {
  asm volatile("s_waitcnt vmcnt(%3)" : "+v"(t.oc), "+v"(t.om), "+v"(t.w) : "n"(YOUNGER) : "memory");
  const bool in = p0 + lane < p1;
  const uint32_t m = in ? t.oc : 0u, v = in ? t.om : 0u;
  t.oc = m * uint32_t(kCoefRow * 4); t.ob = m * row_bytes; t.om = v * mask_bytes;
  t.w = in ? t.w : 0u;
}

struct PLane {
  int kq;
  uint32_t oc, ob, om;
  int mshift;
};

struct POps {
  f32x4 ca[3];
  f32x4 b4, g4;
  uint32_t mw;
  float w;
};

template <bool NOBG> constexpr int kStepLoads = NOBG ? 2 : 6;
template <bool NOBG>
__device__ __forceinline__ void p_load(const PTables& tb, const PMeta& mt, int s, const PLane& pl, POps& o) {
  const int src = 4 * s + pl.kq;
  const uint32_t oc = uint32_t(__shfl(int(mt.oc), src)) + pl.oc;
  const uint32_t om = uint32_t(__shfl(int(mt.om), src)) + pl.om;
  o.w = __uint_as_float(uint32_t(__shfl(int(mt.w), src)));
  bload4<0>(o.ca[0], oc, tb.coef);
  if constexpr (!NOBG) {
    const uint32_t ob = uint32_t(__shfl(int(mt.ob), src)) + pl.ob;
    bload4<kCoefStride * 4>(o.ca[1], oc, tb.coef);
    bload4<2 * kCoefStride * 4>(o.ca[2], oc, tb.coef);
    bload4<0>(o.b4, ob, tb.b);
    bload4<0>(o.g4, ob, tb.g);
  }
  bload1(o.mw, om, tb.mask);
}
template <bool NOBG, int YOUNGER>
__device__ __forceinline__ void p_wait(POps& o) {
  if constexpr (NOBG)
    asm volatile("s_waitcnt vmcnt(%2)" : "+v"(o.ca[0]), "+v"(o.mw) : "n"(YOUNGER) : "memory");
  else
    asm volatile("s_waitcnt vmcnt(%6)" : "+v"(o.ca[0]), "+v"(o.ca[1]), "+v"(o.ca[2]), "+v"(o.b4), "+v"(o.g4), "+v"(o.mw)
                 : "n"(YOUNGER) : "memory");
}

struct PCur { float a1[3], a2[3], bb[4], gg[4]; };
struct PAlpha { u32x4v a[3], m[4]; };
constexpr uint32_t kHiHalves = 0x07060302u;
template <bool NOBG, bool HI, bool SB>
__device__ __forceinline__ void p_xform(const POps& o, const PLane& pl, PCur& c, PAlpha& al, bool bg) {
#pragma unroll
  for (int t = 0; t < 3; ++t) {
    const int tt = HI ? 3 : t;
    if (HI && t > 0) {
      if constexpr (!SB) al.a[t][0] = 0u;
      al.a[t][1] = 0u; al.a[t][2] = 0u;
      continue;
    }
    float av = o.w * o.ca[0][tt];
    asm("" : "+v"(av));
    const uint32_t h0 = __float_as_uint(av) & 0xffff0000u;
    const float r1 = av - __uint_as_float(h0);
    const float r2 = r1 - __uint_as_float(__float_as_uint(r1) & 0xffff0000u);
    if constexpr (!SB) {
      al.a[t][0] = __builtin_amdgcn_perm(__float_as_uint(r1), __float_as_uint(av), kHiHalves);
      al.a[t][1] = __float_as_uint(r2) >> 16;
    } else {
      al.a[t][1] |= h0;
      al.a[t][2] = __builtin_amdgcn_perm(__float_as_uint(r2), __float_as_uint(r1), kHiHalves);
    }
  }
  const int bits = int(o.mw >> pl.mshift);
#pragma unroll
  for (int ct = 0; ct < 4; ++ct) {
    const int on = __builtin_amdgcn_sbfe(bits, ct, 1);
    if constexpr (!SB) {
      al.m[ct][0] = uint32_t(on) & 0x3f803f80u;
      al.m[ct][1] = uint32_t(on) & 0x00003f80u;
    } else {
      al.m[ct][1] |= uint32_t(on) & 0x3f800000u;
      al.m[ct][2] = uint32_t(on) & 0x3f803f80u;
    }
  }
  if constexpr (!NOBG) {
    if (bg) {
#pragma unroll
      for (int t = 0; t < 3; ++t) {
        const int tt = HI ? 3 : t;
        c.a1[t] = (HI && t > 0) ? 0.f : o.w * o.ca[1][tt];
        c.a2[t] = (HI && t > 0) ? 0.f : o.w * o.ca[2][tt];
      }
#pragma unroll
      for (int ct = 0; ct < 4; ++ct) {
        const int on = __builtin_amdgcn_sbfe(bits, ct, 1);
        c.bb[ct] = __uint_as_float(uint32_t(on) & __float_as_uint(o.b4[ct]));
        c.gg[ct] = __uint_as_float(uint32_t(on) & __float_as_uint(o.g4[ct]));
      }
    }
  }
}
template <bool NOBG>
__device__ __forceinline__ void p_keep(const PCur& c) {
  if constexpr (!NOBG) {
    asm volatile("" :: "v"(c.a1[0]), "v"(c.a1[1]), "v"(c.a1[2]), "v"(c.a2[0]), "v"(c.a2[1]), "v"(c.a2[2]));
    asm volatile("" :: "v"(c.bb[0]), "v"(c.bb[1]), "v"(c.bb[2]), "v"(c.bb[3]), "v"(c.gg[0]), "v"(c.gg[1]), "v"(c.gg[2]), "v"(c.gg[3]));
  }
}
__device__ __forceinline__ f32x4 mfma_bf16(u32x4v a, u32x4v b, f32x4 c) {
  return __builtin_amdgcn_mfma_f32_16x16x32_bf16(__builtin_bit_cast(bf16x8, a), __builtin_bit_cast(bf16x8, b), c, 0, 0, 0);
}
__device__ __forceinline__ void p_mfma(const PCur& c, f32x4 (&y2)[3][4]) {
#pragma unroll
  for (int t = 0; t < 3; ++t)
#pragma unroll
    for (int ct = 0; ct < 4; ++ct) y2[t][ct] = __builtin_amdgcn_mfma_f32_16x16x4f32(c.a1[t], c.bb[ct], y2[t][ct], 0, 0, 0);
#pragma unroll
  for (int t = 0; t < 3; ++t)
#pragma unroll
    for (int ct = 0; ct < 4; ++ct) y2[t][ct] = __builtin_amdgcn_mfma_f32_16x16x4f32(c.a2[t], c.gg[ct], y2[t][ct], 0, 0, 0);
}
__device__ __forceinline__ void p_mfma_first(const PCur& c, f32x4 (&y2)[3][4]) {
  const f32x4 zero = {0.f, 0.f, 0.f, 0.f};
#pragma unroll
  for (int t = 0; t < 3; ++t)
#pragma unroll
    for (int ct = 0; ct < 4; ++ct) y2[t][ct] = __builtin_amdgcn_mfma_f32_16x16x4f32(c.a1[t], c.bb[ct], zero, 0, 0, 0);
#pragma unroll
  for (int t = 0; t < 3; ++t)
#pragma unroll
    for (int ct = 0; ct < 4; ++ct) y2[t][ct] = __builtin_amdgcn_mfma_f32_16x16x4f32(c.a2[t], c.gg[ct], y2[t][ct], 0, 0, 0);
}
template <bool FIRST>
__device__ __forceinline__ void p_mfma_alpha(const PAlpha& al, f32x4 (&t1)[3][4]) {
  const f32x4 zero = {0.f, 0.f, 0.f, 0.f};
#pragma unroll
  for (int t = 0; t < 3; ++t)
#pragma unroll
    for (int ct = 0; ct < 4; ++ct) t1[t][ct] = mfma_bf16(al.a[t], al.m[ct], FIRST ? zero : t1[t][ct]);
}

template <bool LIST>
struct ChunkGen {
  int64_t gi;
  int32_t gp, gend;
  int32_t pa0, pa1;
  NodeRanges<LIST> nr;
  __device__ __forceinline__ void init(const int32_t* __restrict__ pptr, const int32_t* __restrict__ list, int64_t n0, int64_t N,
                                       int64_t nn, int64_t cnt) {
    nr.init(pptr, list, n0, N, nn, cnt);
    gi = 0;
    nr.get(0, gp, gend);
    nr.get(1, pa0, pa1);
  }
  __device__ __forceinline__ void next(int64_t cnt, int32_t& q0, int32_t& q1, bool& last) {
    q0 = gp; q1 = min(gp + 64, gend);
    last = q1 >= gend;
    if (last) {
      ++gi;
      gp = pa0; gend = pa1;
      nr.get(gi + 1, pa0, pa1);
    } else {
      gp = q1;
    }
  }
};

template <bool NOBG, bool HI>
__device__ __forceinline__ void pair_body(const PTables& tb, const PMeta& mx, int sx, const PLane& pl, POps& A, POps& B, PCur& cA,
                                          PCur& cB, PAlpha& al, f32x4 (&t1)[3][4], f32x4 (&y2)[3][4], bool first, bool half) {
  constexpr int NL = kStepLoads<NOBG>;
  p_wait<NOBG, NL>(A);
  p_xform<NOBG, HI, false>(A, pl, cA, al, true);
  p_keep<NOBG>(cB);
  p_load<NOBG>(tb, mx, sx, pl, A);
  if constexpr (!NOBG) {
    if (first) p_mfma_first(cA, y2);
    else p_mfma(cA, y2);
  }
  p_wait<NOBG, NL>(B);
  p_xform<NOBG, HI, true>(B, pl, cB, al, !half);
  p_keep<NOBG>(cA);
  p_load<NOBG>(tb, mx, sx + 1, pl, B);
  if (first) p_mfma_alpha<true>(al, t1);
  else p_mfma_alpha<false>(al, t1);
  if constexpr (!NOBG)
    if (!half) p_mfma(cB, y2);
}
template <bool LIST, bool NOBG, bool HI>
__device__ __forceinline__ void product_role(const YArgs& a, const int32_t* __restrict__ pptr, const int32_t* __restrict__ list,
                                             FusedShared& sh, int64_t nn, int64_t cnt, int cg) {
  const int lane = threadIdx.x & 63;
  const int H = a.H;
  const bool path_wave = 64 * cg < H;
  if (!path_wave) return;
  PLane pl;
  const int li = lane & 15;
  pl.kq = lane >> 4;
  const int col = 64 * cg + 4 * li;
  const bool col_ok = col < H;
  pl.oc = 16u * uint32_t(li);
  pl.ob = col_ok ? 4u * uint32_t(col) : 0u;
  pl.om = col_ok ? 4u * uint32_t(col >> 5) : 0x7ffffff0u;
  pl.mshift = col & 31;
  const uint32_t row_bytes = uint32_t(H) * 4u, mask_bytes = uint32_t(a.mask_words) * 4u;
  PTables tb;
  tb.coef = make_rsrc(a.coef, uint64_t(a.n_coef) * kCoefRow * 4);
  tb.b = make_rsrc(a.bg, uint64_t(a.M) * row_bytes);
  tb.g = make_rsrc(a.bg + a.M * int64_t(H), uint64_t(a.M) * row_bytes);
  tb.mask = make_rsrc(a.mask, uint64_t(a.N) * mask_bytes);
  tb.pm = make_rsrc(a.pm, uint64_t(a.cap) * 4);
  tb.pv = make_rsrc(a.pv, uint64_t(a.cap) * 4);
  tb.pw = make_rsrc(a.pw, uint64_t(a.cap) * 4);
  const uint32_t w1_row_bytes = uint32_t(a.w1_ld) * 4u;
  const i32x4 w1rs = make_rsrc(a.W1 + int64_t(a.c0) * a.w1_ld, uint64_t(a.R - 1) * w1_row_bytes + row_bytes);
  constexpr int NL = kStepLoads<NOBG>;
  ChunkGen<LIST> gen;
  gen.init(pptr, list, a.n0, a.N, nn, cnt);
  int32_t q0c, q1c, q0n, q1n;
  bool lastc, lastn;
  gen.next(cnt, q0c, q1c, lastc);
  gen.next(cnt, q0n, q1n, lastn);
  PMeta mc, mn;
  meta_issue(tb, q0c, q1c, lane, mc);
  meta_issue(tb, q0n, q1n, lane, mn);
  meta_finish<0>(q0c, q1c, lane, row_bytes, mask_bytes, mc);
  meta_finish<0>(q0n, q1n, lane, row_bytes, mask_bytes, mn);
  POps A, B;
  p_load<NOBG>(tb, mc, 0, pl, A);
  p_load<NOBG>(tb, mc, 1, pl, B);
  f32x4 t1[3][4], y2[3][4];
#pragma unroll
  for (int t = 0; t < 3; ++t)
#pragma unroll
    for (int ct = 0; ct < 4; ++ct) { t1[t][ct] = f32x4{0.f, 0.f, 0.f, 0.f}; y2[t][ct] = f32x4{0.f, 0.f, 0.f, 0.f}; }
  PCur cA = {}, cB = {};
  PAlpha al;
#pragma unroll
  for (int t = 0; t < 3; ++t) al.a[t] = u32x4v{0u, 0u, 0u, 0u};
#pragma unroll
  for (int ct = 0; ct < 4; ++ct) al.m[ct] = u32x4v{0u, 0u, 0u, 0u};
  bool node_has = false;
  bool firstc = true;
  for (int64_t i = 0; i < cnt;) {
    int32_t q0f, q1f;
    bool lastf;
    gen.next(cnt, q0f, q1f, lastf);
    PMeta mf2;
    meta_issue(tb, q0f, q1f, lane, mf2);
    const int kch = q1c - q0c, np = max((kch + 7) >> 3, 1);
    node_has = node_has || kch > 0;
#pragma clang loop unroll(disable)
    for (int j = 0; j < np; ++j) {
      const bool more = j + 1 < np;
      PMeta mx;
      mx.oc = more ? mc.oc : mn.oc; mx.ob = more ? mc.ob : mn.ob; mx.om = more ? mc.om : mn.om; mx.w = more ? mc.w : mn.w;
      const int sx = more ? 2 * (j + 1) : 0;
      const bool first = firstc && j == 0, half = !more && 4 * (2 * j + 1) >= kch;
      pair_body<NOBG, HI>(tb, mx, sx, pl, A, B, cA, cB, al, t1, y2, first, half);
    }
    if (lastc) {
      int wl = lane;
      asm volatile("" : "+v"(wl));
      const int wkq = wl >> 4, wcol = 64 * cg + 4 * (wl & 15);
      const bool wcol_ok = wcol < H;
      const uint32_t w1_off = wcol_ok ? uint32_t(4 * wkq) * w1_row_bytes + 4u * uint32_t(wcol) : 0x7ff00000u;
      const int pc_lo = 8 * (wcol >> 2) + 4 * piece_swap(wcol >> 2), pc_hi = pc_lo ^ 4;
      f32x4 w1[3][4];
#pragma unroll
      for (int t = 0; t < 3; ++t)
#pragma unroll
        for (int r = 0; r < 4; ++r) bload4<0>(w1[t][r], w1_off + uint32_t(16 * t + r) * w1_row_bytes, w1rs);
      if (i >= 2)
        while (lds_min4(sh.done) < int(i) - 1) __builtin_amdgcn_s_sleep(2);
#pragma unroll
      for (int t = 0; t < 3; ++t)
        asm volatile("s_waitcnt vmcnt(0)" : "+v"(w1[t][0]), "+v"(w1[t][1]), "+v"(w1[t][2]), "+v"(w1[t][3]) :: "memory");
      asm volatile("s_nop 11" ::: "memory");
      __builtin_amdgcn_sched_barrier(0);
      if (node_has && wcol_ok) {
        if (a.gram_f32) {
          float (*ytile)[kYStride] = sh.y[i & 1];
#pragma unroll
          for (int t = 0; t < 3; ++t)
#pragma unroll
            for (int r = 0; r < 4; ++r) {
              f32x4 o;
#pragma unroll
              for (int ct = 0; ct < 4; ++ct) o[ct] = w1[t][r][ct] * t1[t][ct][r] + y2[t][ct][r];
              *reinterpret_cast<f32x4*>(&ytile[16 * t + 4 * wkq + r][wcol]) = o;
            }
        } else {
          uint32_t* __restrict__ grp = &sh.pc[i & 1][wkq][0][0];
#pragma unroll
          for (int t = 0; t < 3; ++t) {
            u32x4v pz[3][2];
#pragma unroll
            for (int ct = 0; ct < 4; ++ct)
#pragma unroll
              for (int rp = 0; rp < 2; ++rp) {
                const float ya = w1[t][2 * rp][ct] * t1[t][ct][2 * rp] + y2[t][ct][2 * rp];
                const float yb = w1[t][2 * rp + 1][ct] * t1[t][ct][2 * rp + 1] + y2[t][ct][2 * rp + 1];
                uint32_t q0, q1, q2;
                split_pair(ya, yb, q0, q1, q2);
                pz[0][ct >> 1][2 * (ct & 1) + rp] = q0;
                pz[1][ct >> 1][2 * (ct & 1) + rp] = q1;
                pz[2][ct >> 1][2 * (ct & 1) + rp] = q2;
              }
            uint32_t* __restrict__ g = grp + 4 * t * kGroupDwords;
            *reinterpret_cast<u32x4v*>(g + pc_lo) = pz[2][0];
            *reinterpret_cast<u32x4v*>(g + pc_hi) = pz[2][1];
            *reinterpret_cast<u32x4v*>(g + kPlaneDwords + pc_lo) = pz[0][0];
            *reinterpret_cast<u32x4v*>(g + kPlaneDwords + pc_hi) = pz[0][1];
            *reinterpret_cast<u32x4v*>(g + 2 * kPlaneDwords + pc_lo) = pz[1][0];
            *reinterpret_cast<u32x4v*>(g + 2 * kPlaneDwords + pc_hi) = pz[1][1];
          }
        }
      }
      ++i;
      lds_publish(&sh.ready[cg], int(i), lane);
#pragma unroll
      for (int t = 0; t < 3; ++t) {
        asm volatile("" : "=v"(t1[t][0]), "=v"(t1[t][1]), "=v"(t1[t][2]), "=v"(t1[t][3]));
        if constexpr (!NOBG) asm volatile("" : "=v"(y2[t][0]), "=v"(y2[t][1]), "=v"(y2[t][2]), "=v"(y2[t][3]));
      }
      node_has = false;
    }
    meta_finish<2 * NL>(q0f, q1f, lane, row_bytes, mask_bytes, mf2);
    firstc = lastc;
    q0c = q0n; q1c = q1n; lastc = lastn; mc = mn;
    q0n = q0f; q1n = q1f; lastn = lastf; mn = mf2;
  }
  asm volatile("s_waitcnt vmcnt(0)" ::: "memory");
}

template <int W>
__device__ __forceinline__ void gram16_load(const float* __restrict__ p, float (&x)[8][2]) {
#pragma unroll
  for (int b = 0; b < 8; ++b) {
    x[b][0] = tiles256_uses<W>(b) ? p[b * 32] : 0.f;
    x[b][1] = tiles256_uses<W>(b) ? p[b * 32 + 16] : 0.f;
  }
}
template <int W>
__device__ __forceinline__ void gram16_mfma(const float (&x)[8][2], f32x4 (&acc)[9][2][2]) {
#pragma unroll
  for (int s = 0; s < 9; ++s)
#pragma unroll
    for (int hi = 0; hi < 2; ++hi)
#pragma unroll
      for (int hj = 0; hj < 2; ++hj) {
        if (Tiles256<W>::si[s] == Tiles256<W>::sj[s] && hi > hj) continue;
        acc[s][hi][hj] = __builtin_amdgcn_mfma_f32_16x16x4f32(x[Tiles256<W>::si[s]][hi], x[Tiles256<W>::sj[s]][hj],
                                                              acc[s][hi][hj], 0, 0, 0);
      }
}
template <int W, bool LIST>
__device__ __forceinline__ void gram_role(const YArgs& a, const int32_t* __restrict__ pptr, const int32_t* __restrict__ list,
                                          FusedShared& sh, int64_t nn, int64_t cnt, float* __restrict__ scratch) {
  const int lane = threadIdx.x & 63;
  f32x4 acc[9][2][2];
#pragma unroll
  for (int s = 0; s < 9; ++s)
#pragma unroll
    for (int q = 0; q < 4; ++q) acc[s][q >> 1][q & 1] = f32x4{0.f, 0.f, 0.f, 0.f};
  const int nk = (a.R + 3) >> 2;
  NodeRanges<LIST> nr;
  nr.init(pptr, list, a.n0, a.N, nn, cnt);
  int32_t p0, p1;
  nr.get(0, p0, p1);
  for (int64_t i = 0; i < cnt; ++i) {
    int32_t q0, q1;
    nr.get(i + 1, q0, q1);
    while (lds_min4(sh.ready) < int(i) + 1) __builtin_amdgcn_s_sleep(2);
    if (p1 > p0) {
      const float* __restrict__ base = &sh.y[i & 1][0][0] + (lane >> 4) * kYStride + (lane & 15);
      float xa[8][2], xb[8][2];
      gram16_load<W>(base, xa);
      for (int kk = 0; kk < nk; kk += 2) {
        if (kk + 1 < nk) gram16_load<W>(base + (kk + 1) * 4 * kYStride, xb);
        __builtin_amdgcn_sched_barrier(0);
        gram16_mfma<W>(xa, acc);
        __builtin_amdgcn_sched_barrier(0);
        if (kk + 1 < nk) {
          if (kk + 2 < nk) gram16_load<W>(base + (kk + 2) * 4 * kYStride, xa);
          __builtin_amdgcn_sched_barrier(0);
          gram16_mfma<W>(xb, acc);
          __builtin_amdgcn_sched_barrier(0);
        }
      }
    }
    lds_publish(&sh.done[W], int(i) + 1, lane);
    p0 = q0; p1 = q1;
  }
  const int64_t D = a.H;
  const int li = lane & 15, lq = lane >> 4;
#pragma unroll
  for (int s = 0; s < 9; ++s)
#pragma unroll
    for (int hi = 0; hi < 2; ++hi)
#pragma unroll
      for (int hj = 0; hj < 2; ++hj) {
        if (Tiles256<W>::si[s] == Tiles256<W>::sj[s] && hi > hj) continue;
        const int64_t jj = Tiles256<W>::sj[s] * 32 + 16 * hj + li;
#pragma unroll
        for (int r = 0; r < 4; ++r) {
          const int64_t ii = Tiles256<W>::si[s] * 32 + 16 * hi + 4 * lq + r;
          if (ii < D && jj < D) atomicAdd(&scratch[ii * D + jj], acc[s][hi][hj][r]);
        }
      }
}

struct PieceBlk { u32x4v t; u32x2v y1; };

template <int W> struct GramOrder;
template <> struct GramOrder<0> { static constexpr int o[9] = {0, 3, 4, 7, 8, 1, 2, 5, 6}; };
template <> struct GramOrder<1> { static constexpr int o[9] = {7, 8, 3, 4, 5, 6, 0, 1, 2}; };
template <> struct GramOrder<2> { static constexpr int o[9] = {7, 8, 3, 4, 5, 6, 0, 1, 2}; };
template <> struct GramOrder<3> { static constexpr int o[9] = {0, 7, 3, 5, 1, 8, 4, 6, 2}; };
template <int W> __device__ __forceinline__ constexpr int gram_last_use(int b) {
  int last = -1;
  for (int p = 0; p < 9; ++p)
    if (Tiles256<W>::si[GramOrder<W>::o[p]] == b || Tiles256<W>::sj[GramOrder<W>::o[p]] == b) last = p;
  return last;
}
template <int W> __device__ __forceinline__ constexpr int gram_first_use(int b) {
  for (int p = 0; p < 9; ++p)
    if (Tiles256<W>::si[GramOrder<W>::o[p]] == b || Tiles256<W>::sj[GramOrder<W>::o[p]] == b) return p;
  return -1;
}

__device__ __forceinline__ void piece_load(const uint32_t* __restrict__ tile, int off, int b, PieceBlk (&x)[8][2]) {
  const uint32_t* __restrict__ pe = tile + off;
  const uint32_t* __restrict__ po = tile + (off ^ 4) + 32;
  const u32x2v e2 = *reinterpret_cast<const u32x2v*>(pe + b * 64), e0 = *reinterpret_cast<const u32x2v*>(pe + kPlaneDwords + b * 64);
  const u32x2v o2 = *reinterpret_cast<const u32x2v*>(po + b * 64), o0 = *reinterpret_cast<const u32x2v*>(po + kPlaneDwords + b * 64);
  x[b][0].t = u32x4v{e2[0], e2[1], e0[0], e0[1]};
  x[b][0].y1 = *reinterpret_cast<const u32x2v*>(pe + 2 * kPlaneDwords + b * 64);
  x[b][1].t = u32x4v{o2[0], o2[1], o0[0], o0[1]};
  x[b][1].y1 = *reinterpret_cast<const u32x2v*>(po + 2 * kPlaneDwords + b * 64);
}
__device__ __forceinline__ u32x4v piece_u(const PieceBlk& p) { return u32x4v{p.t[2], p.t[3], p.y1[0], p.y1[1]}; }
__device__ __forceinline__ u32x4v piece_t(const PieceBlk& p) { return p.t; }
template <int W>
__device__ __forceinline__ void piece_chunk16(PieceBlk (&x)[8][2], f32x4 (&acc)[9][2][2], const uint32_t* __restrict__ tile, int off) {
#pragma unroll
  for (int p = 0; p < 9; ++p) {
    const int s = GramOrder<W>::o[p], si = Tiles256<W>::si[s], sj = Tiles256<W>::sj[s];
#pragma unroll
    for (int b = 0; b < 8; ++b)
      if (gram_first_use<W>(b) == p)
#pragma unroll
        for (int h = 0; h < 2; ++h) asm volatile("" : "+v"(x[b][h].t), "+v"(x[b][h].y1));
    const u32x4v ua[2] = {piece_u(x[si][0]), piece_u(x[si][1])}, ta[2] = {piece_t(x[si][0]), piece_t(x[si][1])};
    const u32x4v ub[2] = {piece_u(x[sj][0]), piece_u(x[sj][1])}, tb[2] = {piece_t(x[sj][0]), piece_t(x[sj][1])};
#pragma unroll
    for (int f = 0; f < 3; ++f)
#pragma unroll
      for (int hi = 0; hi < 2; ++hi)
#pragma unroll
        for (int hj = 0; hj < 2; ++hj) {
          if (si == sj && hi > hj) continue;
          acc[s][hi][hj] = mfma_bf16(f == 1 ? ta[hi] : ua[hi], f == 2 ? tb[hj] : ub[hj], acc[s][hi][hj]);
        }
    __builtin_amdgcn_sched_barrier(0);
#pragma unroll
    for (int b = 0; b < 8; ++b)
      if (gram_last_use<W>(b) == p) piece_load(tile, off, b, x);
  }
}
template <int W>
__device__ __forceinline__ void piece_chunk8(const PieceBlk (&x)[8][2], f32x4 (&acc)[9][2][2], bool low) {
#pragma unroll
  for (int p = 0; p < 9; ++p) {
    const int s = GramOrder<W>::o[p], si = Tiles256<W>::si[s], sj = Tiles256<W>::sj[s];
    u32x4v a1[2], a2[2];
#pragma unroll
    for (int hi = 0; hi < 2; ++hi) {
      const u32x4v u = piece_u(x[si][hi]), t = piece_t(x[si][hi]);
#pragma unroll
      for (int j = 0; j < 4; ++j) { a1[hi][j] = low ? u[j] : t[j]; a2[hi][j] = low ? u[j] : 0u; }
    }
    const u32x4v ub[2] = {piece_u(x[sj][0]), piece_u(x[sj][1])}, tb[2] = {piece_t(x[sj][0]), piece_t(x[sj][1])};
#pragma unroll
    for (int f = 0; f < 2; ++f)
#pragma unroll
      for (int hi = 0; hi < 2; ++hi)
#pragma unroll
        for (int hj = 0; hj < 2; ++hj) {
          if (si == sj && hi > hj) continue;
          acc[s][hi][hj] = mfma_bf16(f == 0 ? a1[hi] : a2[hi], f == 0 ? ub[hj] : tb[hj], acc[s][hi][hj]);
        }
    __builtin_amdgcn_sched_barrier(0);
  }
}
template <int W, bool LIST>
__device__ __forceinline__ void gram_split16_role(const YArgs& a, const int32_t* __restrict__ pptr, const int32_t* __restrict__ list,
                                                  FusedShared& sh, int64_t nn, int64_t cnt, float* __restrict__ scratch) {
  const int lane = threadIdx.x & 63;
  f32x4 acc[9][2][2];
#pragma unroll
  for (int s = 0; s < 9; ++s)
#pragma unroll
    for (int q = 0; q < 4; ++q) acc[s][q >> 1][q & 1] = f32x4{0.f, 0.f, 0.f, 0.f};
  const int n8 = (a.R + 7) >> 3, n16 = n8 >> 1;
  const bool odd = n8 & 1;
  const int gq = lane >> 4;
  const int start = (n16 > 0 ? gq : gq & 1) * kGroupDwords + piece_col(lane & 15);
  const int to_odd = (4 - 2 * (gq >> 1)) * kGroupDwords;
  NodeRanges<LIST> nr;
  nr.init(pptr, list, a.n0, a.N, nn, cnt);
  int32_t p0, p1;
  nr.get(0, p0, p1);
  for (int64_t i = 0; i < cnt; ++i) {
    int32_t q0, q1;
    nr.get(i + 1, q0, q1);
    while (lds_min4(sh.ready) < int(i) + 1) __builtin_amdgcn_s_sleep(2);
    if (p1 > p0) {
      const uint32_t* __restrict__ tile = &sh.pc[i & 1][0][0][0];
      int off = start;
      PieceBlk x[8][2];
#pragma unroll
      for (int b = 0; b < 8; ++b)
        if (tiles256_uses<W>(b)) piece_load(tile, off, b, x);
      __builtin_amdgcn_sched_barrier(0);
      for (int cc = 0; cc < n16; ++cc) {
        off += cc + 1 < n16 ? 4 * kGroupDwords : odd ? to_odd : 0;
        piece_chunk16<W>(x, acc, tile, off);
      }
      if (odd) piece_chunk8<W>(x, acc, gq < 2);
    }
    lds_publish(&sh.done[W], int(i) + 1, lane);
    p0 = q0; p1 = q1;
  }
  const int64_t D = a.H;
  const int fl = int(__builtin_amdgcn_mbcnt_hi(~0u, __builtin_amdgcn_mbcnt_lo(~0u, 0u)));
  const int li = fl & 15, lq = (fl >> 4) & 3;
#pragma unroll
  for (int s = 0; s < 9; ++s)
#pragma unroll
    for (int hi = 0; hi < 2; ++hi)
#pragma unroll
      for (int hj = 0; hj < 2; ++hj) {
        if (Tiles256<W>::si[s] == Tiles256<W>::sj[s] && hi > hj) continue;
        const int64_t jj = Tiles256<W>::sj[s] * 32 + 16 * hj + li;
#pragma unroll
        for (int r = 0; r < 4; ++r) {
          const int64_t ii = Tiles256<W>::si[s] * 32 + 16 * hi + 4 * lq + r;
          if (ii < D && jj < D && (Tiles256<W>::si[s] != Tiles256<W>::sj[s] || ii <= jj)) atomicAdd(&scratch[ii * D + jj], acc[s][hi][hj][r]);
        }
      }
}

template <bool LIST>
__global__ __launch_bounds__(512, 2) void paths_fused_kernel(YArgs a, const int32_t* __restrict__ pptr,
                                                             const int32_t* __restrict__ list, float* __restrict__ scratch) {
  __shared__ FusedShared sh;
  if (int64_t(pptr[a.N]) > a.cap) return;
  for (int q = threadIdx.x; q < int(sizeof(sh.pc) / 16); q += 512) reinterpret_cast<u32x4v*>(&sh.pc[0][0][0][0])[q] = u32x4v{0u, 0u, 0u, 0u};
  if (threadIdx.x < 4) {
    sh.ready[threadIdx.x] = 64 * int(threadIdx.x) < a.H ? 0 : INT32_MAX;
    sh.done[threadIdx.x] = 0;
  }
  __syncthreads();
  const int hw = __builtin_amdgcn_readfirstlane(int(threadIdx.x >> 6));
  const int64_t stride = gridDim.x;
  const int64_t nn = LIST ? int64_t(__builtin_amdgcn_readfirstlane(*a.n_list)) : a.n1 - a.n0;
  const int64_t cnt = nn > int64_t(blockIdx.x) ? (nn - blockIdx.x + stride - 1) / stride : 0;
  switch (hw) {
    case 4: if (a.gram_f32) gram_role<0, LIST>(a, pptr, list, sh, nn, cnt, scratch); else gram_split16_role<0, LIST>(a, pptr, list, sh, nn, cnt, scratch); break;
    case 5: if (a.gram_f32) gram_role<1, LIST>(a, pptr, list, sh, nn, cnt, scratch); else gram_split16_role<1, LIST>(a, pptr, list, sh, nn, cnt, scratch); break;
    case 6: if (a.gram_f32) gram_role<2, LIST>(a, pptr, list, sh, nn, cnt, scratch); else gram_split16_role<2, LIST>(a, pptr, list, sh, nn, cnt, scratch); break;
    case 7: if (a.gram_f32) gram_role<3, LIST>(a, pptr, list, sh, nn, cnt, scratch); else gram_split16_role<3, LIST>(a, pptr, list, sh, nn, cnt, scratch); break;
    default:
      if (a.c0 != a.cb) {
        if (a.no_bg) product_role<LIST, true, true>(a, pptr, list, sh, nn, cnt, hw);
        else product_role<LIST, false, true>(a, pptr, list, sh, nn, cnt, hw);
      } else {
        if (a.no_bg) product_role<LIST, true, false>(a, pptr, list, sh, nn, cnt, hw);
        else product_role<LIST, false, false>(a, pptr, list, sh, nn, cnt, hw);
      }
      break;
  }
}

constexpr int64_t kFusedWorkgroups = 256;

}

int launch_paths_fused(lgnn_ctx* h, YArgs y, int64_t cb, int64_t ce, float* scratch, hipStream_t s) {
  LGNN_REQUIRE(y.N < (int64_t(1) << 31), "too many nodes for one launch");
  const dim3 grid{unsigned(std::min<int64_t>(y.n1 - y.n0, kFusedWorkgroups))};
  const char* e = getenv("LGNN_GRAM_F32");
  y.Y = nullptr; y.gram_f32 = e && atoi(e) != 0 ? 1 : 0;
  for (int64_t c0 = cb; c0 < ce; c0 += kYRows) {
    y.c0 = int(c0); y.R = int(std::min<int64_t>(kYRows, ce - c0));
    if (h->timing) LGNN_CALL(record_event(h, s));
    if (y.list) hipLaunchKernelGGL(paths_fused_kernel<true>, grid, dim3(512), 0, s, y, y.pptr, y.list, scratch);
    else hipLaunchKernelGGL(paths_fused_kernel<false>, grid, dim3(512), 0, s, y, y.pptr, y.list, scratch);
    LGNN_HIP_CHECK(hipGetLastError());
    if (h->timing) { LGNN_CALL(record_event(h, s)); h->ev_planes += y.R; }
  }
  return 0;
}

}
```

Measured before the change: 2.569 million samples/s.

## Replace split-bf16 gram with scaled single-pass f16 gram using runtime bounds

Computes per-column scales of W1 and a runtime magnitude bound from the coefficients, path weights and seed column sums. It then runs the fused gram in a single f16 MFMA pass with power-of-two scaling, unscaling when it flushes the accumulators, instead of the two-piece bf16 split. When the bound falls outside a safe exponent range it falls back to the f32 gram. The aim is fewer MFMA instructions per gram tile. The cost is extra bound and scale kernels, extra atomics in the path-list fill, and a possible loss of precision.

```diff
diff --git a/laplace-gnn_amd/csrc/batchcache.hip b/laplace-gnn_amd/csrc/batchcache.hip
--- a/laplace-gnn_amd/csrc/batchcache.hip
+++ b/laplace-gnn_amd/csrc/batchcache.hip
@@ -158,11 +158,11 @@
   LGNN_REQUIRE(cnt[1] >= 0 && int64_t(cnt[1]) <= std::max<int64_t>(h->nnz, 1) && cnt[2] >= 0 && cnt[2] <= N,
                "internal: path structure counts out of range");
   const size_t nr = size_t(cnt[1]), nn = size_t(cnt[2]);
-  size_t add = size_t(N + 1) * 4 + std::max<size_t>(np, 1) * 12;
+  size_t add = size_t(N + 2) * 4 + std::max<size_t>(np, 1) * 12;
   add += size_t(N + 1) * 4 + std::max<size_t>(nr, 1) * 8;
   if (have_nodes) add += std::max<size_t>(nn, 1) * 4 + 4;
   bool ok = make_room(h, e, add, batch_cache_budget());
-  ok = ok && alloc_copy(e->pptr, ws.path_pptr.p, size_t(N + 1), s) == 0 && alloc_copy(e->pm, ws.path_pm.p, np, s) == 0 &&
+  ok = ok && alloc_copy(e->pptr, ws.path_pptr.p, size_t(N + 2), s) == 0 && alloc_copy(e->pm, ws.path_pm.p, np, s) == 0 &&
        alloc_copy(e->pv, ws.path_pv.p, np, s) == 0 && alloc_copy(e->pw, ws.path_pw.p, np, s) == 0;
   if (ok)
     ok = alloc_copy(e->rptr, ws.path_rptr.p, size_t(N + 1), s) == 0 && alloc_copy(e->r_m, ws.path_rm.p, nr, s) == 0 &&
diff --git a/laplace-gnn_amd/csrc/lgnn_internal.h b/laplace-gnn_amd/csrc/lgnn_internal.h
--- a/laplace-gnn_amd/csrc/lgnn_internal.h
+++ b/laplace-gnn_amd/csrc/lgnn_internal.h
@@ -134,6 +134,8 @@
   DevBuf path_alpha;
   DevBuf path_pcnt, path_pptr, path_pm, path_pv, path_pw;
   DevBuf path_flags, path_nodes, path_nnodes;
+  DevBuf path_scale, path_bgn;
+  DevBuf path_vsum;
   DevBuf pair_s, pair_cnt, pair_ptr, pair_m, pair_m2, pair_w;
   DevBuf pair_part;
   bool path_zeros_set = false;
@@ -156,6 +158,7 @@
     f(act_list); f(act_count); f(select_tmp); f(flags); f(out_flags); f(out_list); f(out_count); f(val_act2);
     f(path_coef); f(path_up); f(path_bg); f(path_cnt); f(path_rptr); f(path_rm); f(path_rw); f(path_zeros); f(path_alpha);
     f(path_pcnt); f(path_pptr); f(path_pm); f(path_pv); f(path_pw); f(path_flags); f(path_nodes); f(path_nnodes);
+    f(path_scale); f(path_bgn); f(path_vsum);
     f(pair_s); f(pair_cnt); f(pair_ptr); f(pair_m); f(pair_m2); f(pair_w); f(pair_part);
     f(planes_c); f(adj_z0); f(adj_dir); f(lora_rows); f(lora_cols); f(lora_state); f(lora_count); f(lora_part);
     f(dense_stored); f(dense_rows);
diff --git a/laplace-gnn_amd/csrc/paths.h b/laplace-gnn_amd/csrc/paths.h
--- a/laplace-gnn_amd/csrc/paths.h
+++ b/laplace-gnn_amd/csrc/paths.h
@@ -31,8 +31,11 @@
   int unused_;
   int no_bg;
   int gram_f32;
+  const float* scale;
 };
-static_assert(sizeof(YArgs) == 240 && __builtin_offsetof(YArgs, no_bg) == 228, "YArgs: paths_fused_kernel's argument offsets");
+static_assert(sizeof(YArgs) == 248 && __builtin_offsetof(YArgs, no_bg) == 228, "YArgs: paths_fused_kernel's argument offsets");
+
+constexpr int kScaleCn = 4, kScaleCinv = kScaleCn + 256, kScaleW1 = kScaleCinv + 256;
 
 struct PathLists {
   const int32_t* rptr; const int32_t* r_m; const float* r_w;
diff --git a/laplace-gnn_amd/csrc/paths.hip b/laplace-gnn_amd/csrc/paths.hip
--- a/laplace-gnn_amd/csrc/paths.hip
+++ b/laplace-gnn_amd/csrc/paths.hip
@@ -4,12 +4,26 @@
 namespace lgnn {
 
 namespace {
+
+__device__ __forceinline__ uint32_t seed_column_sum_max(float al, float be, float ga, float u, float p, int C, int lane) {
+  float vs = 0.f;
+  for (int k = 0; k < C; ++k) {
+    const float uk = __int_as_float(__builtin_amdgcn_readlane(__float_as_int(u), k));
+    const float pk = __int_as_float(__builtin_amdgcn_readlane(__float_as_int(p), k));
+    vs += fabsf((lane == k ? al : 0.f) - be * uk - ga * pk);
+  }
+  uint32_t b = __float_as_uint(vs) & 0x7fffffffu;
+#pragma unroll
+  for (int o = 32; o > 0; o >>= 1) b = max(b, uint32_t(__shfl_xor(int(b), o)));
+  return b;
+}
 
 __global__ __launch_bounds__(256) void path_tables_kernel(const float* __restrict__ probs, const float* __restrict__ logits,
                                                           const int64_t* __restrict__ idx, const int32_t* __restrict__ pos,
                                                           int64_t M, int64_t N, int C, int cb, int ce, int mode,
                                                           float* __restrict__ coef, float* __restrict__ up,
-                                                          const float* __restrict__ W1, int H, float* __restrict__ bg) {
+                                                          const float* __restrict__ W1, int H, float* __restrict__ bg,
+                                                          uint32_t* __restrict__ vsum) {
   const int lane = threadIdx.x & 63;
   const int64_t m = int64_t(blockIdx.x) * 4 + (threadIdx.x >> 6);
   if (m >= M) return;
@@ -37,6 +51,10 @@
   cm[2 * kCoefStride + lane] = have ? -sga : 0.f;
   cm[3 * kCoefStride + lane] = 0.f;
   if (lane < C) { um[lane] = u; pm[lane] = own ? pk : 0.f; }
+  {
+    const uint32_t vb = seed_column_sum_max(al, be, ga, u, own ? pk : 0.f, C, lane);
+    if (lane == 0) vsum[m] = vb;
+  }
   if (bg == nullptr) return;
   const bool colv = 4 * lane < H;
   f32x4 b4 = {0.f, 0.f, 0.f, 0.f}, g4 = {0.f, 0.f, 0.f, 0.f};
@@ -81,6 +99,14 @@
   }
 }
 
+__device__ __forceinline__ void atomic_max_bits(uint32_t* m, uint32_t bits) {
+  if (bits > *reinterpret_cast<volatile uint32_t*>(m)) atomicMax(m, bits);
+}
+__device__ __forceinline__ void path_wsum_max(float wabs, int lane, uint32_t* __restrict__ wsum) {
+  const uint32_t bits = __float_as_uint(wave_sum(wabs)) & 0x7fffffffu;
+  if (lane == 0) atomic_max_bits(wsum, bits);
+}
+
 template <bool FILL>
 __global__ __launch_bounds__(256) void path_list_kernel(const int32_t* __restrict__ rowptr, const int32_t* __restrict__ col,
                                                         const float* __restrict__ val, int64_t N,
@@ -88,7 +114,7 @@
                                                         const float* __restrict__ r_w, int32_t* __restrict__ pcnt,
                                                         const int32_t* __restrict__ pptr, int64_t cap,
                                                         int32_t* __restrict__ pm, int32_t* __restrict__ pv,
-                                                        float* __restrict__ pw) {
+                                                        float* __restrict__ pw, uint32_t* __restrict__ wsum) {
   const int lane = threadIdx.x & 63;
   const int64_t n = int64_t(blockIdx.x) * 4 + (threadIdx.x >> 6);
   if (n >= N) return;
@@ -97,6 +123,7 @@
   }
   const int32_t s = rowptr[n], e = rowptr[n + 1];
   int32_t run = FILL ? pptr[n] : 0;
+  float wabs = 0.f;
   for (int32_t base = s; base < e; base += 64) {
     int32_t v = 0, r0 = 0, cnt = 0;
     float pval = 0.f;
@@ -118,18 +145,20 @@
         pm[off + k] = r_m[r0 + k];
         pv[off + k] = v;
         pw[off + k] = pval * r_w[r0 + k];
+        wabs += fabsf(pval * r_w[r0 + k]);
       }
     }
     run += __shfl(incl, 63);
   }
   if (!FILL && lane == 0) pcnt[n] = run;
+  if constexpr (FILL) path_wsum_max(wabs, lane, wsum);
 }
 
 __global__ __launch_bounds__(256) void sage_path_tables_kernel(const float* __restrict__ probs, const float* __restrict__ logits,
                                                                const int64_t* __restrict__ idx, const int32_t* __restrict__ pos,
                                                                int64_t M, int64_t N, int C, int cb, int ce, int mode,
                                                                float* __restrict__ coef, float* __restrict__ up,
-                                                               float* __restrict__ alpha) {
+                                                               float* __restrict__ alpha, uint32_t* __restrict__ vsum) {
   const int lane = threadIdx.x & 63;
   const int64_t m = int64_t(blockIdx.x) * 4 + (threadIdx.x >> 6);
   if (m >= M + C) return;
@@ -138,6 +167,7 @@
   if (m >= M) {
     float* __restrict__ cm = coef + (2 * M + (m - M)) * kCoefRow;
     cm[lane] = 0.f; cm[kCoefStride + lane] = (have && c == int(m - M)) ? 1.f : 0.f; cm[2 * kCoefStride + lane] = 0.f; cm[3 * kCoefStride + lane] = 0.f;
+    if (lane == 0) vsum[2 * M + (m - M)] = 0u;
     return;
   }
   const int64_t n = idx[m];
@@ -161,6 +191,8 @@
   cn[lane] = sal; cn[kCoefStride + lane] = -sbe; cn[2 * kCoefStride + lane] = -sga; cn[3 * kCoefStride + lane] = 0.f;
   alpha[m * kCoefStride + lane] = al;
   if (lane < C) { up[m * C + lane] = u; up[(M + m) * C + lane] = own ? pk : 0.f; }
+  const uint32_t vb = seed_column_sum_max(al, be, ga, u, own ? pk : 0.f, C, lane);
+  if (lane == 0) { vsum[2 * m] = 0u; vsum[2 * m + 1] = vb; }
 }
 
 template <bool FILL>
@@ -169,12 +201,14 @@
                                                              const int32_t* __restrict__ pos, const int32_t* __restrict__ mult,
                                                              const float* __restrict__ alpha, int32_t* __restrict__ pcnt,
                                                              const int32_t* __restrict__ pptr, int32_t* __restrict__ pm,
-                                                             int32_t* __restrict__ pv, float* __restrict__ pw) {
+                                                             int32_t* __restrict__ pv, float* __restrict__ pw,
+                                                             uint32_t* __restrict__ wsum) {
   const int lane = threadIdx.x & 63;
   const int64_t n = int64_t(blockIdx.x) * 4 + (threadIdx.x >> 6);
   if (n >= N) return;
   const int32_t s = rowptr[n], e = rowptr[n + 1];
   int32_t run = FILL ? pptr[n] : 0;
+  float wabs = 0.f;
   for (int32_t base = s; base < e; base += 64) {
     int32_t mv = INT32_MAX;
     float w = 0.f;
@@ -185,6 +219,7 @@
       if (in) {
         const int32_t o = run + __popcll(bal & ((uint64_t(1) << lane) - 1));
         pm[o] = 2 * mv + 1; pv[o] = int32_t(n); pw[o] = w * float(mult[mv]);
+        wabs += fabsf(w * float(mult[mv]));
       }
     }
     run += __popcll(bal);
@@ -193,15 +228,95 @@
   if (ms != INT32_MAX) {
     if constexpr (FILL) {
       const float tm = float(mult[ms]);
-      if (lane == 0) { pm[run] = 2 * ms; pv[run] = int32_t(n); pw[run] = tm; }
+      if (lane == 0) { pm[run] = 2 * ms; pv[run] = int32_t(n); pw[run] = tm; wabs += tm; }
       if (lane < C) {
         pm[run + 1 + lane] = int32_t(2 * M) + lane; pv[run + 1 + lane] = int32_t(n);
         pw[run + 1 + lane] = tm * alpha[int64_t(ms) * kCoefStride + lane];
+        wabs += fabsf(tm * alpha[int64_t(ms) * kCoefStride + lane]);
       }
     }
     run += 1 + C;
   }
   if (!FILL && lane == 0) pcnt[n] = run;
+  if constexpr (FILL) path_wsum_max(wabs, lane, wsum);
+}
+
+__global__ __launch_bounds__(256) void path_colscale_kernel(const float* __restrict__ W1a, const float* __restrict__ W1b, int ld,
+                                                            int C, int H, float* __restrict__ sc) {
+  const int j = threadIdx.x;
+  uint32_t* __restrict__ bits = reinterpret_cast<uint32_t*>(sc);
+  if (j < 4) bits[j] = 0u;
+  __syncthreads();
+  float va[kCoefStride], vb[kCoefStride];
+#pragma unroll
+  for (int c = 0; c < kCoefStride; ++c) {
+    const bool in = j < H && c < C;
+    va[c] = in ? W1a[int64_t(c) * ld + j] : 0.f;
+    vb[c] = in && W1b ? W1b[int64_t(c) * ld + j] : 0.f;
+  }
+  uint32_t mx = 0u;
+#pragma unroll
+  for (int c = 0; c < kCoefStride; ++c)
+    mx = max(mx, max(__float_as_uint(va[c]) & 0x7fffffffu, __float_as_uint(vb[c]) & 0x7fffffffu));
+  const uint32_t eb = mx >> 23, k = eb == 0u ? 127u : min(max(eb, 1u), 253u);
+  const float cn = __uint_as_float((254u - k) << 23);
+  sc[kScaleCn + j] = cn;
+  sc[kScaleCinv + j] = __uint_as_float(k << 23);
+  uint32_t wm = 0u;
+#pragma unroll
+  for (int c = 0; c < kCoefStride; ++c) {
+    const float v = va[c] * cn;
+    if (j < H && c < C) sc[kScaleW1 + int64_t(c) * H + j] = v;
+    wm = max(wm, max(__float_as_uint(v) & 0x7fffffffu, __float_as_uint(vb[c] * cn) & 0x7fffffffu));
+  }
+  if (wm) atomicMax(&bits[1], wm);
+}
+__global__ __launch_bounds__(256) void path_bound_kernel(const float* __restrict__ coef, int64_t rows, const float* __restrict__ bg,
+                                                         float* __restrict__ bgn, int H, const uint32_t* __restrict__ vsum,
+                                                         float* __restrict__ sc) {
+  const int lane = threadIdx.x & 63, wave = threadIdx.x >> 6;
+  uint32_t amax = 0u, xmax = 0u, vmax = 0u;
+  f32x4 cn = {0.f, 0.f, 0.f, 0.f};
+  if (4 * lane < H) cn = *reinterpret_cast<const f32x4*>(sc + kScaleCn + 4 * lane);
+  for (int64_t r = int64_t(blockIdx.x) * 4 + wave; r < rows; r += int64_t(gridDim.x) * 4) {
+    const f32x4 cf = *reinterpret_cast<const f32x4*>(coef + r * kCoefRow + 4 * lane);
+    uint32_t km = 0u;
+#pragma unroll
+    for (int q = 0; q < 4; ++q) km = max(km, __float_as_uint(cf[q]) & 0x7fffffffu);
+#pragma unroll
+    for (int o = 8; o > 0; o >>= 1) km = max(km, uint32_t(__shfl_xor(int(km), o)));
+    amax = max(amax, uint32_t(__shfl(int(km), 0)));
+    vmax = max(vmax, vsum[r]);
+    if (bg == nullptr) continue;
+    const float be = __uint_as_float(uint32_t(__shfl(int(km), 16))), ga = __uint_as_float(uint32_t(__shfl(int(km), 32)));
+    uint32_t bm = 0u, gm = 0u;
+    if (4 * lane < H) {
+      const f32x4 b4 = *reinterpret_cast<const f32x4*>(bg + r * H + 4 * lane) * cn;
+      const f32x4 g4 = *reinterpret_cast<const f32x4*>(bg + (rows + r) * H + 4 * lane) * cn;
+      *reinterpret_cast<f32x4*>(bgn + r * H + 4 * lane) = b4;
+      *reinterpret_cast<f32x4*>(bgn + (rows + r) * H + 4 * lane) = g4;
+#pragma unroll
+      for (int q = 0; q < 4; ++q) {
+        bm = max(bm, __float_as_uint(b4[q]) & 0x7fffffffu);
+        gm = max(gm, __float_as_uint(g4[q]) & 0x7fffffffu);
+      }
+    }
+#pragma unroll
+    for (int o = 32; o > 0; o >>= 1) {
+      bm = max(bm, uint32_t(__shfl_xor(int(bm), o)));
+      gm = max(gm, uint32_t(__shfl_xor(int(gm), o)));
+    }
+    xmax = max(xmax, __float_as_uint(be * __uint_as_float(bm) + ga * __uint_as_float(gm)) & 0x7fffffffu);
+  }
+  __shared__ uint32_t red[3][4];
+  if (lane == 0) { red[0][wave] = amax; red[1][wave] = xmax; red[2][wave] = vmax; }
+  __syncthreads();
+  if (threadIdx.x < 3) {
+    uint32_t* __restrict__ bits = reinterpret_cast<uint32_t*>(sc);
+    const uint32_t* v = red[threadIdx.x];
+    const int slot = threadIdx.x == 0 ? 0 : int(threadIdx.x) + 1;
+    atomic_max_bits(&bits[slot], max(max(v[0], v[1]), max(v[2], v[3])));
+  }
 }
 
 __global__ void path_flag_kernel(const int32_t* __restrict__ pptr, int64_t n0, int64_t n, uint8_t* __restrict__ flags) {
@@ -295,11 +410,12 @@
 static int path_list_reserve(lgnn_ctx* h, int64_t cap, PathLists& pl, hipStream_t s) {
   Workspace& ws = h->ws;
   LGNN_CALL(ws.path_pcnt.reserve(size_t(h->N + 1) * 4));
-  LGNN_CALL(ws.path_pptr.reserve(size_t(h->N + 1) * 4));
+  LGNN_CALL(ws.path_pptr.reserve(size_t(h->N + 2) * 4));
   LGNN_CALL(ws.path_pm.reserve(size_t(cap) * 4));
   LGNN_CALL(ws.path_pv.reserve(size_t(cap) * 4));
   LGNN_CALL(ws.path_pw.reserve(size_t(cap) * 4));
   LGNN_HIP_CHECK(hipMemsetAsync(ws.path_pcnt.as<int32_t>() + h->N, 0, 4, s));
+  LGNN_HIP_CHECK(hipMemsetAsync(ws.path_pptr.as<int32_t>() + h->N + 1, 0, 4, s));
   pl.pptr = ws.path_pptr.as<int32_t>(); pl.pm = ws.path_pm.as<int32_t>(); pl.pv = ws.path_pv.as<int32_t>();
   pl.pw = ws.path_pw.as<float>();
   return 0;
@@ -321,6 +437,23 @@
   y.mask = h->fc.mask_bits[0].as<uint32_t>(); y.mask_words = int(cdiv(h->dims[1], 32));
   y.N = h->N; y.n0 = nb; y.n1 = ne; y.H = int(h->dims[1]); y.cb = int(cb);
   return y;
+}
+
+static int path_scale_args(lgnn_ctx* h, YArgs& y, const float* W1b, int ld, hipStream_t s) {
+  Workspace& ws = h->ws;
+  const int64_t C = h->dims[2], H = y.H, rows = y.n_coef;
+  LGNN_CALL(ws.path_scale.reserve(size_t(kScaleW1 + C * H) * 4));
+  if (!y.no_bg) LGNN_CALL(ws.path_bgn.reserve(size_t(2 * rows) * H * 4));
+  float* sc = ws.path_scale.as<float>();
+  hipLaunchKernelGGL(path_colscale_kernel, dim3(1), dim3(256), 0, s, y.W1, W1b, ld, int(C), int(H), sc);
+  LGNN_HIP_CHECK(hipGetLastError());
+  hipLaunchKernelGGL(path_bound_kernel, dim3(unsigned(std::min<int64_t>(cdiv(rows, 4), 1024))), dim3(256), 0, s, y.coef, rows,
+                     y.no_bg ? static_cast<const float*>(nullptr) : y.bg, ws.path_bgn.as<float>(), int(H),
+                     ws.path_vsum.as<uint32_t>(), sc);
+  LGNN_HIP_CHECK(hipGetLastError());
+  y.scale = sc; y.W1 = sc + kScaleW1; y.w1_ld = int(H);
+  if (!y.no_bg) y.bg = ws.path_bgn.as<float>();
+  return 0;
 }
 
 int kfac_paths_first_layer(lgnn_ctx* h, const int64_t* idx, int64_t M, int seed_mode, int64_t cb, int64_t ce, float* scratch,
@@ -334,12 +467,13 @@
   LGNN_CALL(ws.path_coef.reserve(size_t(M) * kCoefRow * 4));
   LGNN_CALL(ws.path_up.reserve(size_t(2 * M) * C * 4));
   LGNN_CALL(ws.path_bg.reserve(size_t(2 * M) * H * 4));
+  LGNN_CALL(ws.path_vsum.reserve(size_t(M) * 4));
   const bool no_bg = seed_mode == 2;
   const bool bg_in_tables = !no_bg && (reinterpret_cast<uintptr_t>(h->W[1]) & 15) == 0;
   hipLaunchKernelGGL(path_tables_kernel, dim3(unsigned(cdiv(M, 4))), dim3(256), 0, s, ws.probs.as<float>(),
                      h->fc.out.as<float>(), idx, ws.pos.as<int32_t>(), M, N, int(C), int(cb), int(ce), seed_mode,
                      ws.path_coef.as<float>(), ws.path_up.as<float>(), h->W[1], int(H),
-                     bg_in_tables ? ws.path_bg.as<float>() : static_cast<float*>(nullptr));
+                     bg_in_tables ? ws.path_bg.as<float>() : static_cast<float*>(nullptr), ws.path_vsum.as<uint32_t>());
   LGNN_HIP_CHECK(hipGetLastError());
   if (!no_bg && !bg_in_tables) {
     GemmEpilogue none;
@@ -378,12 +512,13 @@
     hipLaunchKernelGGL(path_list_kernel<false>, pgrid, dim3(256), 0, s, h->PT.rowptr, h->PT.col, h->PT.val, N,
                        ws.path_rptr.as<int32_t>(), ws.path_rm.as<int32_t>(), ws.path_rw.as<float>(), ws.path_pcnt.as<int32_t>(),
                        static_cast<const int32_t*>(nullptr), cap, static_cast<int32_t*>(nullptr), static_cast<int32_t*>(nullptr),
-                       static_cast<float*>(nullptr));
+                       static_cast<float*>(nullptr), static_cast<uint32_t*>(nullptr));
     LGNN_HIP_CHECK(hipGetLastError());
     LGNN_CALL(exclusive_scan_i32(ws.path_pcnt.as<int32_t>(), ws.path_pptr.as<int32_t>(), N + 1, ws.select_tmp, s));
     hipLaunchKernelGGL(path_list_kernel<true>, pgrid, dim3(256), 0, s, h->PT.rowptr, h->PT.col, h->PT.val, N,
                        ws.path_rptr.as<int32_t>(), ws.path_rm.as<int32_t>(), ws.path_rw.as<float>(), ws.path_pcnt.as<int32_t>(),
-                       ws.path_pptr.as<int32_t>(), cap, ws.path_pm.as<int32_t>(), ws.path_pv.as<int32_t>(), ws.path_pw.as<float>());
+                       ws.path_pptr.as<int32_t>(), cap, ws.path_pm.as<int32_t>(), ws.path_pv.as<int32_t>(), ws.path_pw.as<float>(),
+                       ws.path_pptr.as<uint32_t>() + N + 1);
     LGNN_HIP_CHECK(hipGetLastError());
     pl.rptr = ws.path_rptr.as<int32_t>(); pl.r_m = ws.path_rm.as<int32_t>(); pl.r_w = ws.path_rw.as<float>();
   }
@@ -412,7 +547,9 @@
   }
   YArgs y = path_args(h, pl, cb, cap, nb, ne);
   y.W1 = h->W[1]; y.w1_ld = int(H); y.M = M; y.n_coef = M; y.no_bg = no_bg ? 1 : 0;
-  LGNN_CALL(launch_paths_fused(h, y, cb, ce, scratch, s));
+  YArgs yf = y;
+  LGNN_CALL(path_scale_args(h, yf, nullptr, int(H), s));
+  LGNN_CALL(launch_paths_fused(h, yf, cb, ce, scratch, s));
   return can_overflow ? launch_paths_overflow(h, y, cb, ce, scratch, s) : 0;
 }
 
@@ -430,9 +567,10 @@
   LGNN_CALL(ws.path_up.reserve(size_t(2 * M) * C * 4));
   LGNN_CALL(ws.path_bg.reserve(size_t(2 * T) * H * 4));
   LGNN_CALL(ws.path_alpha.reserve(size_t(M) * kCoefStride * 4));
+  LGNN_CALL(ws.path_vsum.reserve(size_t(T) * 4));
   hipLaunchKernelGGL(sage_path_tables_kernel, dim3(unsigned(cdiv(M + C, 4))), dim3(256), 0, s, ws.probs.as<float>(),
                      h->fc.out.as<float>(), idx, ws.pos.as<int32_t>(), M, N, int(C), int(cb), int(ce), seed_mode,
-                     ws.path_coef.as<float>(), ws.path_up.as<float>(), ws.path_alpha.as<float>());
+                     ws.path_coef.as<float>(), ws.path_up.as<float>(), ws.path_alpha.as<float>(), ws.path_vsum.as<uint32_t>());
   LGNN_HIP_CHECK(hipGetLastError());
   float* bg = ws.path_bg.as<float>();
   GemmEpilogue none;
@@ -450,17 +588,19 @@
   hipLaunchKernelGGL(sage_path_list_kernel<false>, pgrid, dim3(256), 0, s, h->PT.rowptr, h->PT.col, h->PT.val, N, M, int(C),
                      ws.pos.as<int32_t>(), ws.mult.as<int32_t>(), ws.path_alpha.as<float>(), ws.path_pcnt.as<int32_t>(),
                      static_cast<const int32_t*>(nullptr), static_cast<int32_t*>(nullptr), static_cast<int32_t*>(nullptr),
-                     static_cast<float*>(nullptr));
+                     static_cast<float*>(nullptr), static_cast<uint32_t*>(nullptr));
   LGNN_HIP_CHECK(hipGetLastError());
   LGNN_CALL(exclusive_scan_i32(ws.path_pcnt.as<int32_t>(), ws.path_pptr.as<int32_t>(), N + 1, ws.select_tmp, s));
   hipLaunchKernelGGL(sage_path_list_kernel<true>, pgrid, dim3(256), 0, s, h->PT.rowptr, h->PT.col, h->PT.val, N, M, int(C),
                      ws.pos.as<int32_t>(), ws.mult.as<int32_t>(), ws.path_alpha.as<float>(), ws.path_pcnt.as<int32_t>(),
-                     ws.path_pptr.as<int32_t>(), ws.path_pm.as<int32_t>(), ws.path_pv.as<int32_t>(), ws.path_pw.as<float>());
+                     ws.path_pptr.as<int32_t>(), ws.path_pm.as<int32_t>(), ws.path_pv.as<int32_t>(), ws.path_pw.as<float>(),
+                     ws.path_pptr.as<uint32_t>() + N + 1);
   LGNN_HIP_CHECK(hipGetLastError());
   LGNN_CALL(path_node_list(h, pl, nb, ne, s));
   YArgs y = path_args(h, pl, cb, cap, nb, ne);
   y.W1 = h->W[1] + H; y.w1_ld = int(2 * H);
   y.M = T; y.n_coef = T; y.no_bg = 0;
+  LGNN_CALL(path_scale_args(h, y, h->W[1], int(2 * H), s));
   return launch_paths_fused(h, y, cb, ce, scratch, s);
 }
 
diff --git a/laplace-gnn_amd/csrc/paths_fused.hip b/laplace-gnn_amd/csrc/paths_fused.hip
--- a/laplace-gnn_amd/csrc/paths_fused.hip
+++ b/laplace-gnn_amd/csrc/paths_fused.hip
@@ -78,18 +78,11 @@
 using u32x4v = __attribute__((ext_vector_type(4))) uint32_t;
 using u32x2v = __attribute__((ext_vector_type(2))) uint32_t;
 
-__device__ __forceinline__ uint32_t pk_bf16(float lo, float hi) {
-  using bf16x2 = __attribute__((ext_vector_type(2))) __bf16;
-  const bf16x2 v = {static_cast<__bf16>(lo), static_cast<__bf16>(hi)};
-  return __builtin_bit_cast(uint32_t, v);
-}
-__device__ __forceinline__ void split_pair(float ya, float yb, uint32_t& q0, uint32_t& q1, uint32_t& q2) {
-  q0 = pk_bf16(ya, yb);
-  asm("" : "+v"(q0));
-  const float r1a = ya - __uint_as_float(q0 << 16), r1b = yb - __uint_as_float(q0 & 0xffff0000u);
-  q1 = pk_bf16(r1a, r1b);
-  asm("" : "+v"(q1));
-  q2 = pk_bf16(r1a - __uint_as_float(q1 << 16), r1b - __uint_as_float(q1 & 0xffff0000u));
+using f16x8 = __attribute__((ext_vector_type(8))) _Float16;
+__device__ __forceinline__ void split_pair(float ya, float yb, uint32_t& h0, uint32_t& h1) {
+  asm("v_cvt_pk_f16_f32 %0, %1, %2" : "=v"(h0) : "v"(ya), "v"(yb));
+  asm("v_fma_mixlo_f16 %0, %1, -1.0, %2 op_sel_hi:[1,0,0]" : "=v"(h1) : "v"(h0), "v"(ya));
+  asm("v_fma_mixhi_f16 %0, %1, -1.0, %2 op_sel:[1,0,0] op_sel_hi:[1,0,0]" : "+v"(h1) : "v"(h0), "v"(yb));
 }
 
 struct PTables {
@@ -104,12 +97,13 @@
   bload1(t.w, q, tb.pw);
 }
 template <int YOUNGER>
-__device__ __forceinline__ void meta_finish(int32_t p0, int32_t p1, int lane, uint32_t row_bytes, uint32_t mask_bytes, PMeta& t) {
+__device__ __forceinline__ void meta_finish(int32_t p0, int32_t p1, int lane, uint32_t row_bytes, uint32_t mask_bytes, float scale,
+                                            PMeta& t) {
   asm volatile("s_waitcnt vmcnt(%3)" : "+v"(t.oc), "+v"(t.om), "+v"(t.w) : "n"(YOUNGER) : "memory");
   const bool in = p0 + lane < p1;
   const uint32_t m = in ? t.oc : 0u, v = in ? t.om : 0u;
   t.oc = m * uint32_t(kCoefRow * 4); t.ob = m * row_bytes; t.om = v * mask_bytes;
-  t.w = in ? t.w : 0u;
+  t.w = in ? __float_as_uint(__uint_as_float(t.w) * scale) : 0u;
 }
 
 struct PLane {
@@ -295,7 +289,7 @@
 }
 template <bool LIST, bool NOBG, bool HI>
 __device__ __forceinline__ void product_role(const YArgs& a, const int32_t* __restrict__ pptr, const int32_t* __restrict__ list,
-                                             FusedShared& sh, int64_t nn, int64_t cnt, int cg) {
+                                             FusedShared& sh, int64_t nn, int64_t cnt, int cg, float scale, bool f32_tile) {
   const int lane = threadIdx.x & 63;
   const int H = a.H;
   const bool path_wave = 64 * cg < H;
@@ -330,8 +324,8 @@
   PMeta mc, mn;
   meta_issue(tb, q0c, q1c, lane, mc);
   meta_issue(tb, q0n, q1n, lane, mn);
-  meta_finish<0>(q0c, q1c, lane, row_bytes, mask_bytes, mc);
-  meta_finish<0>(q0n, q1n, lane, row_bytes, mask_bytes, mn);
+  meta_finish<0>(q0c, q1c, lane, row_bytes, mask_bytes, scale, mc);
+  meta_finish<0>(q0n, q1n, lane, row_bytes, mask_bytes, scale, mn);
   POps A, B;
   p_load<NOBG>(tb, mc, 0, pl, A);
   p_load<NOBG>(tb, mc, 1, pl, B);
@@ -385,7 +379,7 @@
       asm volatile("s_nop 11" ::: "memory");
       __builtin_amdgcn_sched_barrier(0);
       if (node_has && wcol_ok) {
-        if (a.gram_f32) {
+        if (f32_tile) {
           float (*ytile)[kYStride] = sh.y[i & 1];
 #pragma unroll
           for (int t = 0; t < 3; ++t)
@@ -400,22 +394,21 @@
           uint32_t* __restrict__ grp = &sh.pc[i & 1][wkq][0][0];
 #pragma unroll
           for (int t = 0; t < 3; ++t) {
-            u32x4v pz[3][2];
+            u32x4v pz[2][2];
 #pragma unroll
             for (int ct = 0; ct < 4; ++ct)
 #pragma unroll
               for (int rp = 0; rp < 2; ++rp) {
                 const float ya = w1[t][2 * rp][ct] * t1[t][ct][2 * rp] + y2[t][ct][2 * rp];
                 const float yb = w1[t][2 * rp + 1][ct] * t1[t][ct][2 * rp + 1] + y2[t][ct][2 * rp + 1];
-                uint32_t q0, q1, q2;
-                split_pair(ya, yb, q0, q1, q2);
+                uint32_t q0, q1;
+                split_pair(ya, yb, q0, q1);
                 pz[0][ct >> 1][2 * (ct & 1) + rp] = q0;
                 pz[1][ct >> 1][2 * (ct & 1) + rp] = q1;
-                pz[2][ct >> 1][2 * (ct & 1) + rp] = q2;
               }
             uint32_t* __restrict__ g = grp + 4 * t * kGroupDwords;
-            *reinterpret_cast<u32x4v*>(g + pc_lo) = pz[2][0];
-            *reinterpret_cast<u32x4v*>(g + pc_hi) = pz[2][1];
+            *reinterpret_cast<u32x4v*>(g + pc_lo) = pz[1][0];
+            *reinterpret_cast<u32x4v*>(g + pc_hi) = pz[1][1];
             *reinterpret_cast<u32x4v*>(g + kPlaneDwords + pc_lo) = pz[0][0];
             *reinterpret_cast<u32x4v*>(g + kPlaneDwords + pc_hi) = pz[0][1];
             *reinterpret_cast<u32x4v*>(g + 2 * kPlaneDwords + pc_lo) = pz[1][0];
@@ -432,7 +425,7 @@
       }
       node_has = false;
     }
-    meta_finish<2 * NL>(q0f, q1f, lane, row_bytes, mask_bytes, mf2);
+    meta_finish<2 * NL>(q0f, q1f, lane, row_bytes, mask_bytes, scale, mf2);
     firstc = lastc;
     q0c = q0n; q1c = q1n; lastc = lastn; mc = mn;
     q0n = q0f; q1n = q1f; lastn = lastf; mn = mf2;
@@ -440,6 +433,8 @@
   asm volatile("s_waitcnt vmcnt(0)" ::: "memory");
 }
 
+template <int W>
+__device__ __forceinline__ void gram_flush(const YArgs& a, const f32x4 (&acc)[9][2][2], float inv2, float* __restrict__ scratch);
 template <int W>
 __device__ __forceinline__ void gram16_load(const float* __restrict__ p, float (&x)[8][2]) {
 #pragma unroll
@@ -499,25 +494,10 @@
     lds_publish(&sh.done[W], int(i) + 1, lane);
     p0 = q0; p1 = q1;
   }
-  const int64_t D = a.H;
-  const int li = lane & 15, lq = lane >> 4;
-#pragma unroll
-  for (int s = 0; s < 9; ++s)
-#pragma unroll
-    for (int hi = 0; hi < 2; ++hi)
-#pragma unroll
-      for (int hj = 0; hj < 2; ++hj) {
-        if (Tiles256<W>::si[s] == Tiles256<W>::sj[s] && hi > hj) continue;
-        const int64_t jj = Tiles256<W>::sj[s] * 32 + 16 * hj + li;
-#pragma unroll
-        for (int r = 0; r < 4; ++r) {
-          const int64_t ii = Tiles256<W>::si[s] * 32 + 16 * hi + 4 * lq + r;
-          if (ii < D && jj < D) atomicAdd(&scratch[ii * D + jj], acc[s][hi][hj][r]);
-        }
-      }
-}
-
-struct PieceBlk { u32x4v t; u32x2v y1; };
+  gram_flush<W>(a, acc, 1.f, scratch);
+}
+
+struct PieceBlk { u32x4v t; u32x2v h1; };
 
 template <int W> struct GramOrder;
 template <> struct GramOrder<0> { static constexpr int o[9] = {0, 3, 4, 7, 8, 1, 2, 5, 6}; };
@@ -539,17 +519,20 @@
 __device__ __forceinline__ void piece_load(const uint32_t* __restrict__ tile, int off, int b, PieceBlk (&x)[8][2]) {
   const uint32_t* __restrict__ pe = tile + off;
   const uint32_t* __restrict__ po = tile + (off ^ 4) + 32;
-  const u32x2v e2 = *reinterpret_cast<const u32x2v*>(pe + b * 64), e0 = *reinterpret_cast<const u32x2v*>(pe + kPlaneDwords + b * 64);
-  const u32x2v o2 = *reinterpret_cast<const u32x2v*>(po + b * 64), o0 = *reinterpret_cast<const u32x2v*>(po + kPlaneDwords + b * 64);
-  x[b][0].t = u32x4v{e2[0], e2[1], e0[0], e0[1]};
-  x[b][0].y1 = *reinterpret_cast<const u32x2v*>(pe + 2 * kPlaneDwords + b * 64);
-  x[b][1].t = u32x4v{o2[0], o2[1], o0[0], o0[1]};
-  x[b][1].y1 = *reinterpret_cast<const u32x2v*>(po + 2 * kPlaneDwords + b * 64);
-}
-__device__ __forceinline__ u32x4v piece_u(const PieceBlk& p) { return u32x4v{p.t[2], p.t[3], p.y1[0], p.y1[1]}; }
+  const u32x2v e1 = *reinterpret_cast<const u32x2v*>(pe + b * 64), e0 = *reinterpret_cast<const u32x2v*>(pe + kPlaneDwords + b * 64);
+  const u32x2v o1 = *reinterpret_cast<const u32x2v*>(po + b * 64), o0 = *reinterpret_cast<const u32x2v*>(po + kPlaneDwords + b * 64);
+  x[b][0].t = u32x4v{e1[0], e1[1], e0[0], e0[1]};
+  x[b][0].h1 = *reinterpret_cast<const u32x2v*>(pe + 2 * kPlaneDwords + b * 64);
+  x[b][1].t = u32x4v{o1[0], o1[1], o0[0], o0[1]};
+  x[b][1].h1 = *reinterpret_cast<const u32x2v*>(po + 2 * kPlaneDwords + b * 64);
+}
+__device__ __forceinline__ u32x4v piece_u(const PieceBlk& p) { return u32x4v{p.t[2], p.t[3], p.h1[0], p.h1[1]}; }
 __device__ __forceinline__ u32x4v piece_t(const PieceBlk& p) { return p.t; }
+__device__ __forceinline__ f32x4 mfma_f16(u32x4v a, u32x4v b, f32x4 c) {
+  return __builtin_amdgcn_mfma_f32_16x16x32_f16(__builtin_bit_cast(f16x8, a), __builtin_bit_cast(f16x8, b), c, 0, 0, 0);
+}
 template <int W>
-__device__ __forceinline__ void piece_chunk16(PieceBlk (&x)[8][2], f32x4 (&acc)[9][2][2], const uint32_t* __restrict__ tile, int off) {
+__device__ __forceinline__ void piece_chunk16(PieceBlk (&x)[8][2], f32x4 (&acc)[9][2][2], const uint32_t* tile, int off) {
 #pragma unroll
   for (int p = 0; p < 9; ++p) {
     const int s = GramOrder<W>::o[p], si = Tiles256<W>::si[s], sj = Tiles256<W>::sj[s];
@@ -557,17 +540,17 @@
     for (int b = 0; b < 8; ++b)
       if (gram_first_use<W>(b) == p)
 #pragma unroll
-        for (int h = 0; h < 2; ++h) asm volatile("" : "+v"(x[b][h].t), "+v"(x[b][h].y1));
-    const u32x4v ua[2] = {piece_u(x[si][0]), piece_u(x[si][1])}, ta[2] = {piece_t(x[si][0]), piece_t(x[si][1])};
+        for (int h = 0; h < 2; ++h) asm volatile("" : "+v"(x[b][h].t), "+v"(x[b][h].h1));
+    const u32x4v ta[2] = {piece_t(x[si][0]), piece_t(x[si][1])};
     const u32x4v ub[2] = {piece_u(x[sj][0]), piece_u(x[sj][1])}, tb[2] = {piece_t(x[sj][0]), piece_t(x[sj][1])};
 #pragma unroll
-    for (int f = 0; f < 3; ++f)
+    for (int f = 0; f < 2; ++f)
 #pragma unroll
       for (int hi = 0; hi < 2; ++hi)
 #pragma unroll
         for (int hj = 0; hj < 2; ++hj) {
           if (si == sj && hi > hj) continue;
-          acc[s][hi][hj] = mfma_bf16(f == 1 ? ta[hi] : ua[hi], f == 2 ? tb[hj] : ub[hj], acc[s][hi][hj]);
+          acc[s][hi][hj] = mfma_f16(ta[hi], f == 1 ? ub[hj] : tb[hj], acc[s][hi][hj]);
         }
     __builtin_amdgcn_sched_barrier(0);
 #pragma unroll
@@ -576,44 +559,39 @@
   }
 }
 template <int W>
-__device__ __forceinline__ void piece_chunk8(const PieceBlk (&x)[8][2], f32x4 (&acc)[9][2][2], bool low) {
-#pragma unroll
-  for (int p = 0; p < 9; ++p) {
-    const int s = GramOrder<W>::o[p], si = Tiles256<W>::si[s], sj = Tiles256<W>::sj[s];
-    u32x4v a1[2], a2[2];
-#pragma unroll
-    for (int hi = 0; hi < 2; ++hi) {
-      const u32x4v u = piece_u(x[si][hi]), t = piece_t(x[si][hi]);
-#pragma unroll
-      for (int j = 0; j < 4; ++j) { a1[hi][j] = low ? u[j] : t[j]; a2[hi][j] = low ? u[j] : 0u; }
-    }
-    const u32x4v ub[2] = {piece_u(x[sj][0]), piece_u(x[sj][1])}, tb[2] = {piece_t(x[sj][0]), piece_t(x[sj][1])};
-#pragma unroll
-    for (int f = 0; f < 2; ++f)
-#pragma unroll
-      for (int hi = 0; hi < 2; ++hi)
-#pragma unroll
-        for (int hj = 0; hj < 2; ++hj) {
-          if (si == sj && hi > hj) continue;
-          acc[s][hi][hj] = mfma_bf16(f == 0 ? a1[hi] : a2[hi], f == 0 ? ub[hj] : tb[hj], acc[s][hi][hj]);
+__device__ __forceinline__ void gram_flush(const YArgs& a, const f32x4 (&acc)[9][2][2], float inv2, float* __restrict__ scratch) {
+  const int64_t D = a.H;
+  const float* __restrict__ cinv = a.scale + kScaleCinv;
+  const int fl = int(__builtin_amdgcn_mbcnt_hi(~0u, __builtin_amdgcn_mbcnt_lo(~0u, 0u)));
+  const int li = fl & 15, lq = (fl >> 4) & 3;
+#pragma unroll
+  for (int s = 0; s < 9; ++s)
+#pragma unroll
+    for (int hi = 0; hi < 2; ++hi)
+#pragma unroll
+      for (int hj = 0; hj < 2; ++hj) {
+        if (Tiles256<W>::si[s] == Tiles256<W>::sj[s] && hi > hj) continue;
+        const int64_t jj = Tiles256<W>::sj[s] * 32 + 16 * hj + li;
+        const float cj = inv2 * cinv[jj];
+#pragma unroll
+        for (int r = 0; r < 4; ++r) {
+          const int64_t ii = Tiles256<W>::si[s] * 32 + 16 * hi + 4 * lq + r;
+          if (ii < D && jj < D && (Tiles256<W>::si[s] != Tiles256<W>::sj[s] || ii <= jj))
+            atomicAdd(&scratch[ii * D + jj], acc[s][hi][hj][r] * cj * cinv[ii]);
         }
-    __builtin_amdgcn_sched_barrier(0);
-  }
+      }
 }
 template <int W, bool LIST>
-__device__ __forceinline__ void gram_split16_role(const YArgs& a, const int32_t* __restrict__ pptr, const int32_t* __restrict__ list,
-                                                  FusedShared& sh, int64_t nn, int64_t cnt, float* __restrict__ scratch) {
+__device__ __forceinline__ void gram_f16_role(const YArgs& a, const int32_t* __restrict__ pptr, const int32_t* __restrict__ list,
+                                              FusedShared& sh, int64_t nn, int64_t cnt, float inv2, float* __restrict__ scratch) {
   const int lane = threadIdx.x & 63;
   f32x4 acc[9][2][2];
 #pragma unroll
   for (int s = 0; s < 9; ++s)
 #pragma unroll
     for (int q = 0; q < 4; ++q) acc[s][q >> 1][q & 1] = f32x4{0.f, 0.f, 0.f, 0.f};
-  const int n8 = (a.R + 7) >> 3, n16 = n8 >> 1;
-  const bool odd = n8 & 1;
-  const int gq = lane >> 4;
-  const int start = (n16 > 0 ? gq : gq & 1) * kGroupDwords + piece_col(lane & 15);
-  const int to_odd = (4 - 2 * (gq >> 1)) * kGroupDwords;
+  const int n16 = (a.R + 15) >> 4;
+  const int start = (lane >> 4) * kGroupDwords + piece_col(lane & 15);
   NodeRanges<LIST> nr;
   nr.init(pptr, list, a.n0, a.N, nn, cnt);
   int32_t p0, p1;
@@ -623,7 +601,7 @@
     nr.get(i + 1, q0, q1);
     while (lds_min4(sh.ready) < int(i) + 1) __builtin_amdgcn_s_sleep(2);
     if (p1 > p0) {
-      const uint32_t* __restrict__ tile = &sh.pc[i & 1][0][0][0];
+      const uint32_t* tile = &sh.pc[i & 1][0][0][0];
       int off = start;
       PieceBlk x[8][2];
 #pragma unroll
@@ -631,31 +609,27 @@
         if (tiles256_uses<W>(b)) piece_load(tile, off, b, x);
       __builtin_amdgcn_sched_barrier(0);
       for (int cc = 0; cc < n16; ++cc) {
-        off += cc + 1 < n16 ? 4 * kGroupDwords : odd ? to_odd : 0;
+        off += cc + 1 < n16 ? 4 * kGroupDwords : 0;
         piece_chunk16<W>(x, acc, tile, off);
       }
-      if (odd) piece_chunk8<W>(x, acc, gq < 2);
     }
     lds_publish(&sh.done[W], int(i) + 1, lane);
     p0 = q0; p1 = q1;
   }
-  const int64_t D = a.H;
-  const int fl = int(__builtin_amdgcn_mbcnt_hi(~0u, __builtin_amdgcn_mbcnt_lo(~0u, 0u)));
-  const int li = fl & 15, lq = (fl >> 4) & 3;
-#pragma unroll
-  for (int s = 0; s < 9; ++s)
-#pragma unroll
-    for (int hi = 0; hi < 2; ++hi)
-#pragma unroll
-      for (int hj = 0; hj < 2; ++hj) {
-        if (Tiles256<W>::si[s] == Tiles256<W>::sj[s] && hi > hj) continue;
-        const int64_t jj = Tiles256<W>::sj[s] * 32 + 16 * hj + li;
-#pragma unroll
-        for (int r = 0; r < 4; ++r) {
-          const int64_t ii = Tiles256<W>::si[s] * 32 + 16 * hi + 4 * lq + r;
-          if (ii < D && jj < D && (Tiles256<W>::si[s] != Tiles256<W>::sj[s] || ii <= jj)) atomicAdd(&scratch[ii * D + jj], acc[s][hi][hj][r]);
-        }
-      }
+  gram_flush<W>(a, acc, inv2, scratch);
+}
+
+struct GramScale { float s, inv2; bool f32; };
+__device__ __forceinline__ GramScale gram_scale(const YArgs& a, const int32_t* __restrict__ pptr) {
+  const float wsum = __int_as_float(pptr[a.N + 1]);
+  const float tri = a.scale[0] * a.scale[1] + a.scale[2];
+  const float bound = wsum * (fminf(tri, a.scale[3] * a.scale[1]) + 0x1p-12f * tri);
+  const uint32_t eb = __builtin_amdgcn_readfirstlane(int((__float_as_uint(bound) >> 23) & 0x1ffu));
+  GramScale g;
+  g.f32 = a.gram_f32 != 0 || eb < 78u || eb > 204u;
+  g.s = g.f32 ? 1.f : __uint_as_float((268u - eb) << 23);
+  g.inv2 = g.f32 ? 1.f : __uint_as_float((2u * eb - 155u) << 23);
+  return g;
 }
 
 template <bool LIST>
@@ -663,6 +637,7 @@
                                                              const int32_t* __restrict__ list, float* __restrict__ scratch) {
   __shared__ FusedShared sh;
   if (int64_t(pptr[a.N]) > a.cap) return;
+  static_assert(sizeof(sh.pc) >= sizeof(sh.y) && sizeof(sh.pc) % 16 == 0, "the tiles' union");
   for (int q = threadIdx.x; q < int(sizeof(sh.pc) / 16); q += 512) reinterpret_cast<u32x4v*>(&sh.pc[0][0][0][0])[q] = u32x4v{0u, 0u, 0u, 0u};
   if (threadIdx.x < 4) {
     sh.ready[threadIdx.x] = 64 * int(threadIdx.x) < a.H ? 0 : INT32_MAX;
@@ -673,18 +648,19 @@
   const int64_t stride = gridDim.x;
   const int64_t nn = LIST ? int64_t(__builtin_amdgcn_readfirstlane(*a.n_list)) : a.n1 - a.n0;
   const int64_t cnt = nn > int64_t(blockIdx.x) ? (nn - blockIdx.x + stride - 1) / stride : 0;
+  const GramScale gs = gram_scale(a, pptr);
   switch (hw) {
-    case 4: if (a.gram_f32) gram_role<0, LIST>(a, pptr, list, sh, nn, cnt, scratch); else gram_split16_role<0, LIST>(a, pptr, list, sh, nn, cnt, scratch); break;
-    case 5: if (a.gram_f32) gram_role<1, LIST>(a, pptr, list, sh, nn, cnt, scratch); else gram_split16_role<1, LIST>(a, pptr, list, sh, nn, cnt, scratch); break;
-    case 6: if (a.gram_f32) gram_role<2, LIST>(a, pptr, list, sh, nn, cnt, scratch); else gram_split16_role<2, LIST>(a, pptr, list, sh, nn, cnt, scratch); break;
-    case 7: if (a.gram_f32) gram_role<3, LIST>(a, pptr, list, sh, nn, cnt, scratch); else gram_split16_role<3, LIST>(a, pptr, list, sh, nn, cnt, scratch); break;
+    case 4: if (gs.f32) gram_role<0, LIST>(a, pptr, list, sh, nn, cnt, scratch); else gram_f16_role<0, LIST>(a, pptr, list, sh, nn, cnt, gs.inv2, scratch); break;
+    case 5: if (gs.f32) gram_role<1, LIST>(a, pptr, list, sh, nn, cnt, scratch); else gram_f16_role<1, LIST>(a, pptr, list, sh, nn, cnt, gs.inv2, scratch); break;
+    case 6: if (gs.f32) gram_role<2, LIST>(a, pptr, list, sh, nn, cnt, scratch); else gram_f16_role<2, LIST>(a, pptr, list, sh, nn, cnt, gs.inv2, scratch); break;
+    case 7: if (gs.f32) gram_role<3, LIST>(a, pptr, list, sh, nn, cnt, scratch); else gram_f16_role<3, LIST>(a, pptr, list, sh, nn, cnt, gs.inv2, scratch); break;
     default:
       if (a.c0 != a.cb) {
-        if (a.no_bg) product_role<LIST, true, true>(a, pptr, list, sh, nn, cnt, hw);
-        else product_role<LIST, false, true>(a, pptr, list, sh, nn, cnt, hw);
+        if (a.no_bg) product_role<LIST, true, true>(a, pptr, list, sh, nn, cnt, hw, gs.s, gs.f32);
+        else product_role<LIST, false, true>(a, pptr, list, sh, nn, cnt, hw, gs.s, gs.f32);
       } else {
-        if (a.no_bg) product_role<LIST, true, false>(a, pptr, list, sh, nn, cnt, hw);
-        else product_role<LIST, false, false>(a, pptr, list, sh, nn, cnt, hw);
+        if (a.no_bg) product_role<LIST, true, false>(a, pptr, list, sh, nn, cnt, hw, gs.s, gs.f32);
+        else product_role<LIST, false, false>(a, pptr, list, sh, nn, cnt, hw, gs.s, gs.f32);
       }
       break;
   }
@@ -697,6 +673,7 @@
 int launch_paths_fused(lgnn_ctx* h, YArgs y, int64_t cb, int64_t ce, float* scratch, hipStream_t s) {
   LGNN_REQUIRE(y.N < (int64_t(1) << 31), "too many nodes for one launch");
   const dim3 grid{unsigned(std::min<int64_t>(y.n1 - y.n0, kFusedWorkgroups))};
+  LGNN_REQUIRE(y.scale != nullptr, "internal: the fused kernel needs its scale block");
   const char* e = getenv("LGNN_GRAM_F32");
   y.Y = nullptr; y.gram_f32 = e && atoi(e) != 0 ? 1 : 0;
   for (int64_t c0 = cb; c0 < ce; c0 += kYRows) {
```

Measured after the change: 2.758 million samples/s (median of 6 runs). +7.4%, better.
